# xlite-dev/LeetCUDA

Measured on AMD Instinct MI355X. Metric: achieved fp16 TFLOPS vs MI355X MFMA peak: HGEMM 8192^3; FA-2 fwd S=4096 D=128, higher is better.
Workload: dtype f16 (fp32 MFMA accumulate)

## Files before the change

### include/lc_diag.h

```cpp
#ifndef LC_DIAG_H_
#define LC_DIAG_H_

#ifdef __cplusplus
extern "C" {
#endif

int lc_probe_mfma16(const void* a16x32, const void* b16x32, float* d16x16, void* stream);
int lc_probe_mfma32(const void* a32x16, const void* b32x16, float* d32x32, void* stream);
int lc_probe_tr16(const void* src_64x4_u16, void* dst_64x4_u16, void* stream);
int lc_probe_coissue(int filler, int k, int mode, void* out_u64x16, void* stream);
int lc_probe_attn_mix(int waves, int mix, void* out_u64x16, void* stream);
int lc_diag_attn_w4u_stamps(const void* Q, const void* K, const void* V, void* O, void* lse, int B, int H, int N, int nsplit, void* out_u64x16,
                            void* stream);
int lc_probe_mfma_form(int form, void* out_u64x16, void* stream);
int lc_probe_mfma_war(int delay, int kind, int queued, const void* a32x16, const void* b32x16, float* d32x32,
                      void* stream);

int lc_diag_pollute(unsigned pattern, int what, void* stream);

int lc_diag_attn_w4i(int abl, const void* Q, const void* K, const void* V, void* O, int B, int H, int N, int D, void* stream);

int lc_probe_mid256(const void* A, const void* B, void* C, int M, int N, int K, int b_kn, int panel_w, void* stream);

#ifdef __cplusplus
}
#endif
#endif
```

### leetcuda_amd/build.py

```python
from __future__ import annotations

import argparse
import json
import os
import shutil
import subprocess
import sys
from pathlib import Path

ROOT = Path(__file__).resolve().parent.parent
PKG = ROOT / "leetcuda_amd"
CSRC = PKG / "csrc"
LIBDIR = PKG / "lib"
ORACLE = ROOT / "oracle"
ROCM = Path(os.environ.get("ROCM_PATH", "/opt/rocm"))

LIB_NAME = "libleetcuda_amd.so"
ORACLE_NAME = "liblc_oracle.so"


def _newer(target: Path, sources) -> bool:
    if not target.exists():
        return False
    t = target.stat().st_mtime
    return all(Path(s).stat().st_mtime <= t for s in sources)


def _digest(paths, extra="") -> str:
    import hashlib
    h = hashlib.sha256(extra.encode())
    for q in sorted(Path(x) for x in paths):
        h.update(str(q.relative_to(ROOT) if q.is_relative_to(ROOT) else q).encode())
        h.update(q.read_bytes() if q.exists() else b"<missing>")
    return h.hexdigest()


def _stamps() -> dict:
    try:
        return json.loads((LIBDIR / "stamps.json").read_text())
    except Exception:
        return {}


def _fresh(target: Path, key: str, digest: str) -> bool:
    return target.exists() and _stamps().get(key) == digest


def _mark(key: str, digest: str):
    LIBDIR.mkdir(parents=True, exist_ok=True)
    st = _stamps()
    st[key] = digest
    (LIBDIR / "stamps.json").write_text(json.dumps(st, indent=1))


def _run(cmd, **kw):
    print("[build]", " ".join(str(c) for c in cmd), flush=True)
    subprocess.run([str(c) for c in cmd], check=True, **kw)


def hipcc() -> str:
    exe = shutil.which("hipcc") or str(ROCM / "bin" / "hipcc")
    if not Path(exe).exists():
        raise RuntimeError("hipcc not found: the MI355X kernels cannot be built")
    return exe


def _flags():
    diag = os.environ.get("LC_DIAG") == "1"
    return ["--offload-arch=gfx950", "-O3", "-std=c++17", "-fPIC", "-Wno-unused-result", "-fno-honor-nans",
            "-mno-amdgpu-ieee", *(["-DLC_DIAG"] if diag else []), f"-I{ROOT / 'include'}"]


def _portable(flags):
    return [str(f).replace(str(ROOT), "$ROOT") for f in flags]


def _stamp_ok(stamp: Path, flags) -> bool:
    try:
        return json.loads(stamp.read_text())["flags"] == _portable(flags)
    except Exception:
        return False


def _unit_deps(dep: Path):
    txt = dep.read_text().replace("\\\n", " ")
    return [Path(d) for d in (txt.split(":", 1)[1].split() if ":" in txt else [])]


def _unit_digest(dep: Path, flags) -> str:
    import hashlib
    h = hashlib.sha256(" ".join(_portable(flags)).encode())
    for q in sorted(_unit_deps(dep), key=lambda x: (x.name, str(x))):
        h.update(q.name.encode())
        h.update(q.read_bytes() if q.exists() else b"<missing>")
    return h.hexdigest()


def _unit_current(obj: Path, asm, dep: Path, flags) -> bool:
    if not obj.exists() or not dep.exists() or (asm is not None and not asm.exists()):
        return False
    deps = _unit_deps(dep)
    if not deps or not all(d.exists() for d in deps):
        return False
    have = _stamps().get("unit:" + obj.stem)
    if have is None:
        return False
    return have == _unit_digest(dep, flags)


def build_abi(force: bool = False, audit: bool = True) -> Path:
    LIBDIR.mkdir(parents=True, exist_ok=True)
    out = LIBDIR / LIB_NAME
    stamp = LIBDIR / "build_stamp.json"
    srcs = sorted(CSRC.glob("*.hip")) + sorted(CSRC.glob("*.h")) + sorted(CSRC.glob("*.inc"))
    srcs.append(ROOT / "include" / "lc_abi.h")
    srcs.append(PKG / "isa_audit.py")
    srcs.append(ROOT / "tools" / "gen_hgemm_w4y.py")
    srcs.append(ROOT / "tools" / "gen_attn_w4i.py")
    srcs.append(ROOT / "tools" / "gen_gemm_fp8_w4k.py")
    srcs.append(ROOT / "tools" / "gen_attn_bigd7.py")
    flags = _flags()
    gen = subprocess.run([sys.executable, str(ROOT / "tools" / "gen_hgemm_w4y.py"), "--check"], capture_output=True, text=True)
    if gen.returncode != 0:
        raise RuntimeError("generated sources are stale: " + gen.stderr.strip())
    for script in ("gen_attn_w4i.py", "gen_gemm_fp8_w4k.py", "gen_attn_bigd7.py"):
        gen = subprocess.run([sys.executable, str(ROOT / "tools" / script), "--check"], capture_output=True, text=True)
        if gen.returncode != 0:
            raise RuntimeError("generated sources are stale: " + gen.stderr.strip())
    if os.environ.get("LC_DIAG") == "1":
        subprocess.run([sys.executable, str(ROOT / "tools" / "gen_hgemm_w4y.py"), "--diag", str(LIBDIR / "gen")], check=True)
        flags = flags + [f"-I{LIBDIR / 'gen'}"]
    dg = _digest(srcs, " ".join(_portable(flags)))
    if not force and _fresh(out, "abi", dg) and _stamp_ok(stamp, flags):
        return out
    objdir = LIBDIR / "obj"
    objdir.mkdir(exist_ok=True)
    units = [CSRC / "lc_abi.hip"] + sorted(CSRC.glob("tu_*.hip"))
    for old in list(objdir.glob("tu_*.*")):
        if old.suffix in (".o", ".s", ".d") and not (CSRC / (old.stem + ".hip")).exists():
            old.unlink()
    flags_ok = _stamp_ok(stamp, flags)
    procs = []
    for u in units:
        obj = objdir / (u.stem + ".o")
        asm = objdir / (u.stem + ".s")
        dep = objdir / (u.stem + ".d")
        if not force and flags_ok and _unit_current(obj, asm if audit else None, dep, flags):
            procs.append((u, obj, None))
            continue
        for stale in (obj, asm):
            if stale.exists():
                stale.unlink()
        cmd = [hipcc(), *flags, "-MD", "-MF", str(dep), "-c", "-o", str(obj), str(u)]
        print("[build] " + " ".join(cmd), flush=True)
        procs.append((u, obj, subprocess.Popen(cmd, stdout=subprocess.PIPE, stderr=subprocess.STDOUT, text=True)))
        if audit:
            cmd = [hipcc(), *flags, "-S", "--cuda-device-only", "-Wno-unused-command-line-argument", "-o", str(asm), str(u)]
            procs.append((u, None, subprocess.Popen(cmd, stdout=subprocess.PIPE, stderr=subprocess.STDOUT, text=True)))
    objs = []
    for u, obj, pr in procs:
        if pr is not None:
            log, _ = pr.communicate()
            if pr.returncode != 0:
                sys.stdout.write(log[-8000:])
                raise subprocess.CalledProcessError(pr.returncode, pr.args)
        if obj is not None:
            objs.append(obj)
            if pr is not None:
                _mark("unit:" + obj.stem, _unit_digest(objdir / (obj.stem + ".d"), flags))
    if audit:
        from leetcuda_amd import isa_audit
        reps, bad = isa_audit.audit_files([objdir / (u.stem + ".s") for u in units])
        for r in reps:
            print(f"[audit] {r.name}: vgpr {r.vgpr_count} agpr {r.agpr_count} scratch {r.scratch} "
                  f"asm loads {r.asm_loads} compiler v_accvgpr {r.compiler_accvgpr}", flush=True)
        (objdir / "isa_audit.json").write_text(json.dumps(
            [{"kernel": r.name, "vgpr": r.vgpr_count, "agpr": r.agpr_count, "scratch": r.scratch,
              "asm_loads": r.asm_loads, "compiler_accvgpr": r.compiler_accvgpr, "violations": r.violations}
             for r in reps], indent=1))
        if bad:
            if out.exists():
                out.unlink()
            raise RuntimeError("ISA audit failed (leetcuda_amd/isa_audit.py):\n  " + "\n  ".join(bad))
    _run([hipcc(), "--offload-arch=gfx950", "-shared", "-fPIC", "-o", out, *objs, "-ldl"])
    stamp.write_text(json.dumps({"flags": _portable(flags)}))
    _mark("abi", dg)
    return out


def build_diag(force: bool = False) -> Path:
    LIBDIR.mkdir(parents=True, exist_ok=True)
    out = LIBDIR / "liblc_diag.so"
    srcs = sorted((CSRC / "diag").glob("*.hip")) + [CSRC / "lc_common.h", ROOT / "include" / "lc_diag.h", CSRC / "attn_w4i.hip", CSRC / "attn_w4u.hip", CSRC / "attn_w4u_body.inc", CSRC / "attn_mp.h", CSRC / "attn_fwd.hip", CSRC / "attn_fwd_body.inc",
                                                     CSRC / "hgemm_mid.hip", ROOT / "tools" / "gen_attn_w4i.py"]
    dg = _digest(srcs)
    if not force and _fresh(out, "diag", dg):
        return out
    gen = LIBDIR / "gen"
    subprocess.run([sys.executable, str(ROOT / "tools" / "gen_attn_w4i.py"), "--diag", str(gen)], check=True)
    sys.path.insert(0, str(ROOT / "tools"))
    try:
        import gen_attn_w4i
        abls = gen_attn_w4i.ABLATIONS
    finally:
        sys.path.pop(0)
    objdir = LIBDIR / "obj"
    objdir.mkdir(exist_ok=True)
    base = [hipcc(), "--offload-arch=gfx950", "-O3", "-std=c++17", "-fPIC", "-Wno-unused-result", "-Wno-inline-asm",
            "-fno-honor-nans", "-mno-amdgpu-ieee", f"-I{ROOT / 'include'}", f"-I{gen}", f"-I{CSRC}"]
    jobs = [(objdir / "diag_main.o", [*base, "-c", "-o", objdir / "diag_main.o", CSRC / "diag" / "lc_diag.hip"]),
            (objdir / "diag_w4u_stamps.o", [*base, "-c", "-o", objdir / "diag_w4u_stamps.o", CSRC / "diag" / "attn_w4u_stamps.hip"]),
            (objdir / "diag_mid256.o", [*base, "-c", "-o", objdir / "diag_mid256.o", CSRC / "diag" / "mid256_probe.hip"])]
    for k in abls:
        o = objdir / f"diag_w4i_abl{k}.o"
        jobs.append((o, [*base, f"-DW4I_ABL={k}", f'-DW4I_INC32="attn_w4i_d32_abl{k}.inc"', f'-DW4I_INC64="attn_w4i_d64_abl{k}.inc"', f'-DW4I_INC96="attn_w4i_d96_abl{k}.inc"', f'-DW4I_INC128="attn_w4i_d128_abl{k}.inc"',
                         "-c", "-o", o, CSRC / "diag" / "attn_w4i_abl.hip"]))
    procs = []
    for o, cmd in jobs:
        print("[build]", " ".join(str(c) for c in cmd), flush=True)
        procs.append((o, subprocess.Popen([str(c) for c in cmd], stdout=subprocess.PIPE, stderr=subprocess.STDOUT, text=True)))
    for o, pr in procs:
        log, _ = pr.communicate()
        if pr.returncode != 0:
            sys.stdout.write(log[-6000:])
            raise subprocess.CalledProcessError(pr.returncode, pr.args)
    _run([hipcc(), "--offload-arch=gfx950", "-shared", "-fPIC", "-o", out, *[o for o, _ in jobs]])
    _mark("diag", dg)
    return out


def build_cpp_bench(force: bool = False) -> Path:
    d = ROOT / "tools" / "cpp"
    out = d / "hgemm_bench.bin"
    build_abi(False)
    dg = _digest([d / "hgemm_bench.cpp", d / "Makefile", ROOT / "include" / "lc_abi.h"])
    if not force and _fresh(out, "cpp_bench", dg):
        return out
    _run(["make", "-C", d, "-B"])
    _mark("cpp_bench", dg)
    return out


def build_oracle(force: bool = False) -> Path:
    out = ORACLE / ORACLE_NAME
    srcs = [ORACLE / "lc_oracle.c", ORACLE / "lc_oracle.h"]
    dg = _digest(srcs)
    if not force and _fresh(out, "oracle", dg):
        return out
    cc = shutil.which("gcc") or "cc"
    _run([cc, "-O3", "-mavx2", "-mfma", "-fopenmp", "-fPIC", "-shared", "-std=c11", "-o", out,
          ORACLE / "lc_oracle.c", "-lm"])
    _mark("oracle", dg)
    return out


def build_torch_ext(force: bool = False):
    import sysconfig

    import torch
    from torch.utils import cpp_extension

    suffix = sysconfig.get_config_var("EXT_SUFFIX") or ".so"
    outs = []
    abi = build_abi(force=False)
    inc = [f"-I{p}" for p in cpp_extension.include_paths()] + [f"-I{ROOT / 'include'}"]
    inc += [f"-I{sysconfig.get_paths()['include']}", f"-I{ROCM / 'include'}"]
    torch_lib = Path(torch.__file__).parent / "lib"
    cxx = shutil.which("g++") or "c++"
    for name in ("toy_hgemm", "flash_attn_lib"):
        src = CSRC / "torch" / f"{name}.cpp"
        out = PKG / f"{name}{suffix}"
        dg = _digest([src, CSRC / "torch" / "torch_shim.h", ROOT / "include" / "lc_abi.h"], extra="rpath: $ORIGIN/lib, $ORIGIN/leetcuda_amd/lib")
        if not force and _fresh(out, f"torch_{name}", dg):
            outs.append(out)
            continue
        cmd = [cxx, "-O2", "-std=c++17", "-fPIC", "-shared", "-D__HIP_PLATFORM_AMD__=1",
               "-DUSE_ROCM=1", f"-DTORCH_EXTENSION_NAME={name}", "-DTORCH_API_INCLUDE_EXTENSION_H",
               f"-D_GLIBCXX_USE_CXX11_ABI={int(torch._C._GLIBCXX_USE_CXX11_ABI)}", *inc, src, "-o", out,
               f"-L{LIBDIR}", "-lleetcuda_amd", "-Wl,-rpath,$ORIGIN/lib", "-Wl,-rpath,$ORIGIN/leetcuda_amd/lib", f"-L{torch_lib}",
               "-lc10", "-lc10_hip", "-ltorch", "-ltorch_cpu", "-ltorch_hip", "-ltorch_python",
               f"-Wl,-rpath,{torch_lib}"]
        _run(cmd)
        _mark(f"torch_{name}", dg)
        outs.append(out)
    return outs


def build_all(force: bool = False, torch_ext: bool = True):
    abi = build_abi(force)
    build_diag(force)
    build_cpp_bench(force)
    orc = build_oracle(force)
    ext = build_torch_ext(force) if torch_ext else []
    return abi, orc, ext


if __name__ == "__main__":
    ap = argparse.ArgumentParser()
    ap.add_argument("--force", action="store_true")
    ap.add_argument("--no-torch-ext", action="store_true")
    a = ap.parse_args()
    res = build_all(a.force, not a.no_torch_ext)
    print("[build] ok:", res)
    sys.exit(0)
```

### leetcuda_amd/capi.py

```python
from __future__ import annotations

import ctypes as C
import os
from pathlib import Path

_PKG = Path(__file__).resolve().parent
LIB_PATH = _PKG / "lib" / "libleetcuda_amd.so"
DIAG_LIB_PATH = _PKG / "lib" / "liblc_diag.so"

LC_OK, LC_ERR_ARG, LC_ERR_SHAPE, LC_ERR_HEADDIM, LC_ERR_LAUNCH, LC_ERR_VENDOR, LC_ERR_DEVICE = 0, -1, -2, -3, -4, -5, -6
LAYOUT_NN, LAYOUT_TN = 0, 1
HGEMM_AUTO, HGEMM_MFMA256, HGEMM_GENERIC, HGEMM_MFMA256P2, HGEMM_MFMA128 = 0, 1, 3, 4, 6
HGEMM_VALU_NAIVE, HGEMM_VALU_SLICED_K, HGEMM_VALU_T8X8_X4, HGEMM_VALU_T16X8_K32 = 20, 21, 22, 30
HGEMM_MFMA256W4B, HGEMM_MFMA256W4C, HGEMM_MFMA256W4X, HGEMM_MFMA256W4Y = 9, 10, 12, 13
HGEMM_MID = 14
HGEMM_EDGE = 15
HGEMM_RAGGED = 16
HGEMM_KPAD = 17
ATTN_SPLIT_Q, ATTN_SHARED_QKV, ATTN_SHARED_KV, ATTN_TILING_QK, ATTN_TILING_QKV, ATTN_SPLIT_KV = range(6)
ATTN_CAUSAL, ATTN_V_TRANSPOSED = 1, 2

_vp, _i, _cp, _fp, _ip = C.c_void_p, C.c_int, C.c_char_p, C.POINTER(C.c_float), C.POINTER(C.c_int)
SYMBOLS = {
    "lc_abi_version": (_i, []),
    "lc_status_string": (_cp, [_i]),
    "lc_device_check": (_i, [_ip]),
    "lc_build_info": (_cp, [_ip]),
    "lc_tune_set": (_i, [_cp, _i]),
    "lc_tune_get": (_i, [_cp, _ip, _ip]),
    "lc_tune_count": (_i, []),
    "lc_tune_key": (_cp, [_i]),
    "lc_tune_calibrate": (_i, [_vp, _fp]),
    "lc_workspace_release": (C.c_size_t, []),
    "lc_workspace_bytes": (C.c_size_t, []),
    "lc_hgemm_f16": (_i, [_vp, _vp, _vp, _i, _i, _i, _i, _i, _i, _i, _vp]),
    "lc_vendor_init": (_i, []),
    "lc_vendor_destroy": (_i, []),
    "lc_hgemm_vendor_f16": (_i, [_vp, _vp, _vp, _i, _i, _i, _i, _vp]),
    "lc_gemm_fp8_e4m3": (_i, [_vp, _vp, _vp, _i, _i, _i, C.c_float, _i, _vp]),
    "lc_mxfp8_pack_scales": (_i, [_vp, _vp, _i, _i, _vp]),
    "lc_gemm_mxfp8": (_i, [_vp, _vp, _vp, _vp, _vp, _i, _i, _i, C.c_float, _i, _vp]),
    "lc_hgemm_call": (_i, [_cp, _vp, _vp, _vp, _i, _i, _i, _i, _i, _i, _vp]),
    "lc_hgemm_entry_count": (_i, []),
    "lc_hgemm_entry_name": (_cp, [_i]),
    "lc_hgemm_entry_info": (_i, [_cp, _ip, _ip]),
    "lc_attn_fwd_f16": (_i, [_vp, _vp, _vp, _vp, _i, _i, _i, _i, _i, _i, _i, _i, _vp]),
    "lc_attn_fwd_bf16": (_i, [_vp, _vp, _vp, _vp, _i, _i, _i, _i, _vp]),
    "lc_attn_fwd_f16_ex": (_i, [_vp, _vp, _vp, _vp, _i, _i, _i, _i, _i, _vp]),
    "lc_attn_call": (_i, [_cp, _vp, _vp, _vp, _vp, _i, _i, _i, _i, _i, _vp]),
    "lc_attn_entry_count": (_i, []),
    "lc_attn_entry_name": (_cp, [_i]),
    "lc_attn_entry_info": (_i, [_cp, _ip, _ip, _ip, _ip, _ip, _ip]),
    "lc_hgemm_time": (_i, [_vp, _vp, _vp, _i, _i, _i, _i, _i, _i, _i, _i, _i, _vp, _fp]),
    "lc_attn_time": (_i, [_vp, _vp, _vp, _vp, _i, _i, _i, _i, _i, _i, _i, _i, _i, _vp, _fp]),
    "lc_hgemm_kernel_name": (_i, [_i, _i, _i, _i, _i, _cp, _i]),
    "lc_attn_kernel_name": (_i, [_i, _i, _i, _i, _cp, _i]),
    "lc_attn_kernel_name_bh": (_i, [_i, _i, _i, _i, _i, _cp, _i]),
    "lc_attn_kernel_name_ex": (_i, [_i, _i, _i, _i, _cp, _i]),
    "lc_attn_slowpath_stats": (_i, [C.POINTER(C.c_uint), _i]),
    "lc_timer_start": (_i, [_vp, C.POINTER(_vp)]),
    "lc_timer_stop": (_i, [_vp, _fp]),
    "lc_clock_probe": (_i, [_vp, _vp]),
}
DIAG_SYMBOLS = {
    "lc_probe_mid256": (_i, [_vp, _vp, _vp, _i, _i, _i, _i, _i, _vp]),
    "lc_probe_mfma16": (_i, [_vp, _vp, _vp, _vp]),
    "lc_probe_mfma32": (_i, [_vp, _vp, _vp, _vp]),
    "lc_probe_tr16": (_i, [_vp, _vp, _vp]),
    "lc_probe_coissue": (_i, [_i, _i, _i, _vp, _vp]),
    "lc_probe_attn_mix": (_i, [_i, _i, _vp, _vp]),
    "lc_probe_mfma_form": (_i, [_i, _vp, _vp]),
    "lc_probe_mfma_war": (_i, [_i, _i, _i, _vp, _vp, _vp, _vp]),
    "lc_diag_pollute": (_i, [C.c_uint, _i, _vp]),
    "lc_diag_attn_w4i": (_i, [_i, _vp, _vp, _vp, _vp, _i, _i, _i, _i, _vp]),
    "lc_diag_attn_w4u_stamps": (_i, [_vp, _vp, _vp, _vp, _vp, _i, _i, _i, _i, _vp, _vp]),
}

_lib = None
_diag = None


class LcError(RuntimeError):
    def __init__(self, status: int, what: str):
        self.status = status
        super().__init__(f"{what}: {status_string(status)} (lc_status {status})")


def load() -> C.CDLL:
    global _lib
    if _lib is not None:
        return _lib
    if not LIB_PATH.exists():
        raise RuntimeError(
            f"{LIB_PATH} is missing: build it with `python -m leetcuda_amd.build` "
            "(there is no CPU or PyTorch fallback for the HIP kernels)")
    try:
        import torch
        tl = Path(torch.__file__).parent / "lib" / "libhipblaslt.so"
        if tl.exists() and os.environ.get("LC_VENDOR_SYSTEM_HIPBLASLT", "0") != "1":
            C.CDLL(str(tl), mode=C.RTLD_GLOBAL)
    except Exception:
        pass
    lib = C.CDLL(str(LIB_PATH), mode=C.RTLD_GLOBAL)
    for name, (res, args) in SYMBOLS.items():
        fn = getattr(lib, name)
        fn.restype, fn.argtypes = res, args
    _lib = lib
    return lib


def load_diag() -> C.CDLL:
    global _diag
    if _diag is not None:
        return _diag
    if not DIAG_LIB_PATH.exists():
        raise RuntimeError(f"{DIAG_LIB_PATH} is missing: build it with `python -m leetcuda_amd.build`")
    import torch
    lib = C.CDLL(str(DIAG_LIB_PATH), mode=C.RTLD_GLOBAL)
    for name, (res, args) in DIAG_SYMBOLS.items():
        fn = getattr(lib, name)
        fn.restype, fn.argtypes = res, args
    _diag = lib
    return lib


def build_info():
    d = C.c_int(0)
    return load().lc_build_info(C.byref(d)).decode(), bool(d.value)


def require_production():
    info, diag = build_info()
    if diag:
        raise RuntimeError(f"libleetcuda_amd.so is a DIAGNOSIS build ({info}); rebuild with "
                           "`python -m leetcuda_amd.build --force` (LC_DIAG unset)")


def status_string(status: int) -> str:
    return load().lc_status_string(status).decode()


def check(status: int, what: str):
    if status != LC_OK:
        raise LcError(status, what)


def _ptr(t) -> int:
    return t.data_ptr()


def _stream() -> int:
    import torch
    return torch.cuda.current_stream().cuda_stream


def _shape_err(what: str):
    raise RuntimeError(f"Tensor size mismatch! ({what})")


def _gemm_dims(a, b, c, layout=LAYOUT_NN, b_is_nk=False):
    if a.dim() != 2 or b.dim() != 2 or c.dim() != 2:
        _shape_err("2-D tensors expected")
    M, K = a.shape
    N = c.shape[1]
    if c.shape[0] != M:
        _shape_err(f"c {tuple(c.shape)} vs a {tuple(a.shape)}")
    if b_is_nk:
        ok = tuple(b.shape) == (N, K)
    elif layout == LAYOUT_TN:
        ok = tuple(b.shape) in ((K, N), (N, K))
    else:
        ok = tuple(b.shape) == (K, N)
    if not ok:
        _shape_err(f"b {tuple(b.shape)} vs K={K}, N={N}")
    return M, N, K


def _attn_dims(q, k, v, o, v_transposed=False):
    if q.dim() != 4:
        _shape_err("4-D [B,H,N,D] tensors expected")
    B, H, N, D = q.shape
    vshape = (B, H, D, N) if v_transposed else (B, H, N, D)
    if tuple(k.shape) != (B, H, N, D) or tuple(o.shape) != (B, H, N, D) or tuple(v.shape) != vshape:
        _shape_err(f"q {tuple(q.shape)} k {tuple(k.shape)} v {tuple(v.shape)} o {tuple(o.shape)}")
    return B, H, N, D


def _need_gpu(*tensors):
    for t in tensors:
        if not t.is_cuda:
            raise RuntimeError("leetcuda_amd: tensor must live on the MI355X (no CPU path)")
        if not t.is_contiguous():
            raise RuntimeError("leetcuda_amd: tensor must be contiguous")


def tune(key: str, value: int):
    check(load().lc_tune_set(key.encode(), value), f"lc_tune_set({key})")


def tune_get(key: str):
    v, d = C.c_int(0), C.c_int(0)
    check(load().lc_tune_get(key.encode(), C.byref(v), C.byref(d)), f"lc_tune_get({key})")
    return v.value, d.value


def tune_items():
    lib = load()
    out = {}
    for i in range(lib.lc_tune_count()):
        k = lib.lc_tune_key(i)
        if k:
            out[k.decode()] = tune_get(k.decode())
    return out


def tune_calibrate():
    out = (C.c_float * 4)()
    rc = load().lc_tune_calibrate(_stream(), out)
    if rc not in (LC_OK, LC_ERR_ARG):
        check(rc, "lc_tune_calibrate")
    return {"adopted": rc == LC_OK, "tau128_us": out[0], "tau64_us": out[1], "x0_us": out[2], "bytes_per_us": out[3]}


def workspace_bytes() -> int:
    return int(load().lc_workspace_bytes())


def workspace_release() -> int:
    return int(load().lc_workspace_release())


def device_check() -> int:
    n = C.c_int(0)
    check(load().lc_device_check(C.byref(n)), "lc_device_check")
    return n.value


def hgemm(a, b, c, layout=LAYOUT_NN, variant=HGEMM_AUTO, stages=2, swizzle_stride=1):
    import torch
    _need_gpu(a, b, c)
    assert a.dtype == b.dtype == c.dtype == torch.half
    M, N, K = _gemm_dims(a, b, c, layout)
    check(load().lc_hgemm_f16(_ptr(a), _ptr(b), _ptr(c), M, N, K, layout, variant, stages, swizzle_stride,
                              _stream()), "lc_hgemm_f16")
    return c


def gemm_fp8(a8, b8_nk, c, alpha=1.0, swizzle_stride=1):
    _need_gpu(a8, b8_nk, c)
    M, N, K = _gemm_dims(a8, b8_nk, c, b_is_nk=True)
    check(load().lc_gemm_fp8_e4m3(_ptr(a8), _ptr(b8_nk), _ptr(c), M, N, K, float(alpha), swizzle_stride, _stream()),
          "lc_gemm_fp8_e4m3")
    return c


def mxfp8_pack_scales(s):
    import torch
    _need_gpu(s)
    assert s.dtype == torch.uint8 and s.dim() == 2 and s.is_contiguous()
    rows, kb = s.shape
    p = torch.empty(rows * kb, dtype=torch.uint8, device=s.device)
    check(load().lc_mxfp8_pack_scales(_ptr(s), _ptr(p), rows, kb * 32, _stream()), "lc_mxfp8_pack_scales")
    return p


def gemm_mxfp8(a8, pa, b8_nk, pb, c, alpha=1.0, swizzle_stride=1):
    _need_gpu(a8, b8_nk, c, pa, pb)
    M, N, K = _gemm_dims(a8, b8_nk, c, b_is_nk=True)
    assert pa.numel() == M * K // 32 and pb.numel() == N * K // 32
    check(load().lc_gemm_mxfp8(_ptr(a8), _ptr(pa), _ptr(b8_nk), _ptr(pb), _ptr(c), M, N, K, float(alpha), swizzle_stride, _stream()),
          "lc_gemm_mxfp8")
    return c


def hgemm_call(entry: str, a, b, c, stages=2, swizzle=False, swizzle_stride=1):
    _need_gpu(a, b, c)
    lay = C.c_int(LAYOUT_NN)
    load().lc_hgemm_entry_info(entry.encode(), C.byref(lay), None)
    M, N, K = _gemm_dims(a, b, c, lay.value)
    check(load().lc_hgemm_call(entry.encode(), _ptr(a), _ptr(b), _ptr(c), M, N, K, stages, int(swizzle),
                               swizzle_stride, _stream()), entry)
    return c


def hgemm_vendor(a, b, c, layout=LAYOUT_NN):
    _need_gpu(a, b, c)
    M, N, K = _gemm_dims(a, b, c, layout)
    check(load().lc_hgemm_vendor_f16(_ptr(a), _ptr(b), _ptr(c), M, N, K, layout, _stream()),
          "lc_hgemm_vendor_f16")
    return c


def vendor_init():
    check(load().lc_vendor_init(), "lc_vendor_init")


def vendor_destroy():
    check(load().lc_vendor_destroy(), "lc_vendor_destroy")


def hgemm_time(a, b, c, layout=LAYOUT_NN, variant=HGEMM_AUTO, stages=2, swizzle_stride=1, warmup=2,
               iters=10) -> float:
    _need_gpu(a, b, c)
    M, N, K = _gemm_dims(a, b, c, layout)
    ms = C.c_float(0)
    check(load().lc_hgemm_time(_ptr(a), _ptr(b), _ptr(c), M, N, K, layout, variant, stages, swizzle_stride,
                               warmup, iters, _stream(), C.byref(ms)), "lc_hgemm_time")
    return ms.value


def hgemm_entries():
    lib = load()
    out = []
    for i in range(lib.lc_hgemm_entry_count()):
        name = lib.lc_hgemm_entry_name(i)
        lay, na = C.c_int(), C.c_int()
        lib.lc_hgemm_entry_info(name, C.byref(lay), C.byref(na))
        out.append((name.decode(), lay.value, na.value))
    return out


def attn_fwd(q, k, v, o, v_transposed=False, family=ATTN_SPLIT_Q, acc_f32=False, stages=2, causal=False):
    import torch
    _need_gpu(q, k, v, o)
    assert q.dtype == k.dtype == v.dtype == o.dtype == torch.half
    B, H, N, D = _attn_dims(q, k, v, o, v_transposed)
    if causal:
        flags = ATTN_CAUSAL | (ATTN_V_TRANSPOSED if v_transposed else 0)
        check(load().lc_attn_fwd_f16_ex(_ptr(q), _ptr(k), _ptr(v), _ptr(o), B, H, N, D, flags, _stream()), "lc_attn_fwd_f16_ex")
        return o
    check(load().lc_attn_fwd_f16(_ptr(q), _ptr(k), _ptr(v), _ptr(o), B, H, N, D, int(v_transposed), family,
                                 int(acc_f32), stages, _stream()), "lc_attn_fwd_f16")
    return o


def attn_fwd_bf16(q, k, v, o):
    import torch
    _need_gpu(q, k, v, o)
    assert q.dtype == k.dtype == v.dtype == o.dtype == torch.bfloat16
    B, H, N, D = _attn_dims(q, k, v, o)
    check(load().lc_attn_fwd_bf16(_ptr(q), _ptr(k), _ptr(v), _ptr(o), B, H, N, D, _stream()), "lc_attn_fwd_bf16")
    return o


def attn_call(entry: str, q, k, v, o, stages=2):
    _need_gpu(q, k, v, o)
    vt = C.c_int(0)
    load().lc_attn_entry_info(entry.encode(), None, C.byref(vt), None, None, None, None)
    B, H, N, D = _attn_dims(q, k, v, o, bool(vt.value))
    check(load().lc_attn_call(entry.encode(), _ptr(q), _ptr(k), _ptr(v), _ptr(o), B, H, N, D, stages,
                              _stream()), entry)
    return o


def attn_time(q, k, v, o, v_transposed=False, family=ATTN_SPLIT_Q, stages=2, warmup=1, iters=5) -> float:
    _need_gpu(q, k, v, o)
    B, H, N, D = _attn_dims(q, k, v, o, v_transposed)
    ms = C.c_float(0)
    check(load().lc_attn_time(_ptr(q), _ptr(k), _ptr(v), _ptr(o), B, H, N, D, int(v_transposed), family,
                              stages, warmup, iters, _stream(), C.byref(ms)), "lc_attn_time")
    return ms.value


def attn_entries():
    lib = load()
    out = []
    for i in range(lib.lc_attn_entry_count()):
        name = lib.lc_attn_entry_name(i)
        v = [C.c_int() for _ in range(6)]
        lib.lc_attn_entry_info(name, *[C.byref(x) for x in v])
        out.append((name.decode(),) + tuple(x.value for x in v))
    return out


class Timer:

    def __enter__(self):
        self._t = C.c_void_p()
        check(load().lc_timer_start(_stream(), C.byref(self._t)), "lc_timer_start")
        self.ms = None
        return self

    def __exit__(self, et, ev, tb):
        ms = C.c_float(0)
        rc = load().lc_timer_stop(self._t, C.byref(ms))
        if et is None:
            check(rc, "lc_timer_stop")
            self.ms = ms.value
        return False


def hgemm_kernel_name(M, N, K, layout=LAYOUT_NN, variant=HGEMM_AUTO) -> str:
    buf = C.create_string_buffer(128)
    check(load().lc_hgemm_kernel_name(M, N, K, layout, variant, buf, 128), "lc_hgemm_kernel_name")
    return buf.value.decode()


def attn_slowpath_stats(reset=True):
    import struct
    out = (C.c_uint * 4)()
    check(load().lc_attn_slowpath_stats(out, int(reset)), "lc_attn_slowpath_stats")
    return [out[0], out[1], out[2], struct.unpack("f", struct.pack("I", out[3]))[0]]


def attn_kernel_name(N, D, v_transposed=False, bf16=False, bh=None, causal=False) -> str:
    buf = C.create_string_buffer(128)
    if causal:
        assert not bf16, "causal attention is fp16 only"
        flags = ATTN_CAUSAL | (ATTN_V_TRANSPOSED if v_transposed else 0)
        check(load().lc_attn_kernel_name_ex(int(bh) if bh else -1, N, D, flags, buf, 128), "lc_attn_kernel_name_ex")
        return buf.value.decode()
    check(load().lc_attn_kernel_name_bh(int(bh) if bh else -1, N, D, int(v_transposed), int(bf16), buf, 128), "lc_attn_kernel_name_bh")
    return buf.value.decode()


def clock_probe(out_u64x2):
    check(load().lc_clock_probe(_ptr(out_u64x2), _stream()), "lc_clock_probe")
```

### leetcuda_amd/csrc/hgemm_w4y.hip

```cpp
#pragma once
#include "hgemm_w4x.hip"

namespace lc {

struct W4yNNSrc {
  const char* ub;
  unsigned b_off[2];
  unsigned bq, bkt;
};
LC_DEVINL void w4y_nn_src_init(W4yNNSrc& s, const half_t* B, int n0, int N, int wave, int lane) {
  const int pp = lane & 15, kr = lane >> 4;
#pragma unroll
  for (int par = 0; par < 2; ++par) {
    const int pair = (pp >> 1) ^ ((kr << 1) | par);
    s.b_off[par] = (unsigned)kr * (unsigned)N * 2u + (unsigned)((pair * 2 + (pp & 1)) * 16);
  }
  s.ub = (const char*)(B + (size_t)(wave * 16) * N + n0);
  s.bq = (unsigned)N * 8u;
  s.bkt = (unsigned)N * 128u;
}

template <bool ALPHA = false>
LC_DEVINL void w4y_epilogue_b2(char* slot, half_t* C, int N, int m0, int n0, int wave, int wr, int wc, int lane, float alpha = 1.f) {
  asm volatile("" : "+v"(lane));
  const int r16 = lane & 15, kg = lane >> 4;
  char* stg = slot + wave * (32 * 256);
  half_t* cw = C + (size_t)(m0 + wr * 128) * N + n0 + wc * 128;
  static_for<4>([&](auto qc) {
    constexpr int q = decltype(qc)::value;
    static_for<4>([&](auto gc) {
      constexpr int ih = decltype(gc)::value >> 1, j0 = 4 * (decltype(gc)::value & 1);
      constexpr int blk = 8 * (2 * q + ih) + j0;
      float x[16];
      acc_read16<4 * blk, 4 * (blk + 1), 4 * (blk + 2), 4 * (blk + 3)>(x);
#pragma unroll
      for (int jj = 0; jj < 4; ++jj) {
        const int j = j0 + jj;
        half4_t h;
        if constexpr (ALPHA) {
          h[0] = (half_t)(alpha * x[4 * jj + 0]);
          h[1] = (half_t)(alpha * x[4 * jj + 1]);
          h[2] = (half_t)(alpha * x[4 * jj + 2]);
          h[3] = (half_t)(alpha * x[4 * jj + 3]);
        } else {
          h[0] = (half_t)x[4 * jj + 0];
          h[1] = (half_t)x[4 * jj + 1];
          h[2] = (half_t)x[4 * jj + 2];
          h[3] = (half_t)x[4 * jj + 3];
        }
        *(half4_t*)(stg + (16 * ih + r16) * 256 + (((2 * j + (kg >> 1)) ^ r16) * 16) + 8 * (kg & 1)) = h;
      }
    });
    asm volatile("s_waitcnt lgkmcnt(0)" ::: "memory");
#pragma unroll
    for (int it = 0; it < 8; ++it) {
      const int row = it * 4 + (lane >> 4);
      const u32x4_t v = *(const u32x4_t*)(stg + row * 256 + (((lane & 15) ^ (row & 15)) * 16));
      *(u32x4_t*)(cw + (size_t)(q * 32 + row) * N + (lane & 15) * 8) = v;
    }
    asm volatile("s_waitcnt lgkmcnt(0)" ::: "memory");
  });
}

template <int BLK0, int BLK1>
LC_DEVINL void w4y_tail_mfma2(half8_t b0, half8_t b1, half8_t a) {
  asm volatile("s_nop 1\n\tv_mfma_f32_16x16x32_f16 a[%3:%4], %0, %2, a[%3:%4]\n\tv_mfma_f32_16x16x32_f16 a[%5:%6], %1, %2, a[%5:%6]"
               :: "v"(b0), "v"(b1), "v"(a), "n"(BLK0 * 4), "n"(BLK0 * 4 + 3), "n"(BLK1 * 4), "n"(BLK1 * 4 + 3)
               : LC_AGPR_ALL);
}
template <bool B_KN>
LC_DEVINL void w4y_k_tail(const half_t* __restrict__ A, const half_t* __restrict__ B, int N, int K, int k0, int mw, int nw, int lane) {
  asm volatile("" : "+v"(lane), "+s"(N), "+s"(K));
  const int r16 = lane & 15, kg = lane >> 4;
  const half_t* ap = A + ((size_t)(mw + r16) * K + k0 + 8 * kg);
  half8_t xb[8];
  if constexpr (!B_KN) {
    const half_t* bp = B + ((size_t)(nw + r16) * K + k0 + 8 * kg);
#pragma unroll
    for (int j = 0; j < 8; ++j) xb[j] = *(const half8_t*)(bp + (size_t)16 * j * K);
  } else {
    const half_t* bp = B + ((size_t)(k0 + 8 * kg) * N + nw + r16);
#pragma unroll
    for (int e = 0; e < 8; ++e) {
      const half_t* be = bp + (size_t)e * N;
#pragma unroll
      for (int j = 0; j < 8; ++j) xb[j][e] = be[16 * j];
    }
  }
  static_for<8>([&](auto ic) {
    constexpr int i = decltype(ic)::value;
    const half8_t xa = *(const half8_t*)(ap + (size_t)16 * i * K);
    static_for<4>([&](auto jc) {
      constexpr int jp = decltype(jc)::value;
      w4y_tail_mfma2<8 * i + 2 * jp, 8 * i + 2 * jp + 1>(xb[2 * jp], xb[2 * jp + 1], xa);
    });
  });
}

template <bool B_KN, int SCHED>
__global__ __launch_bounds__(256) void hgemm_w4y_kernel(const half_t* __restrict__ A, const half_t* __restrict__ B,
                                                       half_t* __restrict__ C, int M, int N, int K, int tiles_m,
                                                       int tiles_n, int panel_w, int stagger, int ntiles) {
  extern __shared__ __attribute__((aligned(16))) char smem[];
  const int lane = threadIdx.x & 63;
  const int wave = wave_id();
  const int wr = wave >> 1, wc = wave & 1;

  int vb = __builtin_amdgcn_readfirstlane((int)blockIdx.x);
  const int vstride = __builtin_amdgcn_readfirstlane((int)gridDim.x);
  const int nvb = ntiles > 0 ? ntiles : vstride;
  const int KT = K / BK;

  W4Src<false> src;
  w4_src_init<false>(src, A, B, 0, 0, N, K, wave, lane);
  src.a_off[0] = src.a_off[1] = (wave & 1) ? src.a_off[1] : src.a_off[0];
  src.a_blk = (size_t)32 * K * 2;
  W4yNNSrc nsrc;
  if constexpr (B_KN) w4y_nn_src_init(nsrc, B, 0, N, wave, lane);

  struct TileCtx {
    int m0, n0;
    const char* ua;
    const char* ub;
    uint32_t stg;
  };
  auto tile_ctx = [&](int v) -> TileCtx {
    const TileCoord tc = block_tile(v, nvb, tiles_m, tiles_n, panel_w);
    TileCtx c;
    c.m0 = tc.tm * BM;
    c.n0 = tc.tn * BN;
    c.ua = (const char*)(A + (size_t)(c.m0 + wave * 8) * K);
    c.ub = B_KN ? (const char*)(B + (size_t)(wave * 16) * N + c.n0) : (const char*)(B + (size_t)(c.n0 + wave * 8) * K);
    const int cx = stagger & 15, cm = (stagger >> 4) & 15, cn = (stagger >> 8) & 15, step = (stagger >> 12) & 0xff, mask = (stagger >> 20) & 0x7f;
    const int idx = cx * (v & 7) + cm * __builtin_amdgcn_readfirstlane(tc.tm) + cn * __builtin_amdgcn_readfirstlane(tc.tn);
    c.stg = (uint32_t)__builtin_amdgcn_readfirstlane((int)((unsigned)((idx & mask) * step) % (unsigned)KT));
    return c;
  };
  auto a_slot = [&](int t) -> char* { return smem + (t & 1) * TILE_BYTES; };
  auto b_slot = [&](int bi) -> char* { return smem + (2 + bi) * TILE_BYTES; };
  auto issue_prologue = [&](const TileCtx& c) {
    const buf_rsrc_t ra = make_rsrc(c.ua), rb = make_rsrc(c.ub);
    auto piece = [&](int g, int t, char* slot) {
      int te = (t < KT ? t : KT - 1) + (int)c.stg;
      if (te >= KT) te -= KT;
      if (g < 8) {
        blds16(ra, src.a_off[0], (unsigned)((size_t)g * src.a_blk + (size_t)te * src.a_kt), slot + g * 4096 + wave * 1024);
      } else if constexpr (!B_KN) {
        blds16(rb, src.a_off[0], (unsigned)((size_t)(g - 8) * src.a_blk + (size_t)te * src.b_kt),
               slot + (g - 8) * 4096 + wave * 1024);
      } else {
        const int p = g - 8, h = p >> 2, p2 = p & 3;
        blds16(rb, nsrc.b_off[(p2 >> 1) & 1], (unsigned)p2 * nsrc.bq + 256u * h + (unsigned)te * nsrc.bkt,
               slot + h * HALF_BYTES + (wave * 4 + p2) * 1024);
      }
    };
#pragma unroll
    for (int g = 8; g < 16; ++g) piece(g, 0, b_slot(0));
#pragma unroll
    for (int g = 0; g < 8; ++g) piece(g, 0, a_slot(0));
#pragma unroll
    for (int g = 8; g < 16; ++g) piece(g, 1, b_slot(1));
#pragma unroll
    for (int g = 0; g < 8; ++g) piece(g, 1, a_slot(1));
  };

  W4xFrag fr;
  w4x_frag_init(fr, wr, wc, lane);

  TileCtx cur = tile_ctx(vb);
  issue_prologue(cur);
  for (;;) {
  static_for<256>([&](auto r) { w4_acc_zero<decltype(r)::value>(); });
  LC_VMCNT(16);
  pp_barrier();
  const int m0 = cur.m0, n0 = cur.n0;
  const uint32_t w4y_stg = cur.stg;
  const char* ubp = cur.ub;

  {
    const uint64_t pa = (uint64_t)cur.ua, pb = (uint64_t)ubp;
    const u32x4_t w4y_ra = {(uint32_t)__builtin_amdgcn_readfirstlane((uint32_t)pa),
                            (uint32_t)__builtin_amdgcn_readfirstlane((uint32_t)(pa >> 32)) & 0xffffu, 0x7fffffffu, 0x00020000u};
    const u32x4_t w4y_rb = {(uint32_t)__builtin_amdgcn_readfirstlane((uint32_t)pb),
                            (uint32_t)__builtin_amdgcn_readfirstlane((uint32_t)(pb >> 32)) & 0xffffu, 0x7fffffffu, 0x00020000u};
    const uint32_t w4y_a0 = __builtin_amdgcn_readfirstlane(lds_addr32(smem));
    const uint32_t w4y_wv = (uint32_t)wave * 1024u;
    const uint32_t w4y_blk = __builtin_amdgcn_readfirstlane((uint32_t)src.a_blk);
    const uint32_t w4y_ao0 = src.a_off[0], w4y_ao1 = src.a_off[1];
    uint32_t w4y_t, w4y_acur, w4y_anxt, w4y_b0, w4y_b1, w4y_b2, w4y_soff, w4y_t2off, w4y_tmp, w4y_swp;
    if constexpr (B_KN) {
      const uint32_t w4y_wvb = (uint32_t)wave * 4096u;
      const uint32_t w4y_bq = __builtin_amdgcn_readfirstlane(nsrc.bq), w4y_bkt = __builtin_amdgcn_readfirstlane(nsrc.bkt);
      const uint32_t w4y_bo0 = nsrc.b_off[0], w4y_bo1 = nsrc.b_off[1];
      const int ti = lane & 15, tg = lane >> 4;
      const uint32_t w4y_bk = (uint32_t)(wc * HALF_BYTES + (8 * tg + (ti >> 2)) * 256 + (ti & 3) * 8);
      const uint32_t w4y_key = (uint32_t)(((ti >> 2) << 1) | (tg & 1));
      uint32_t w4y_t2offb;
#include "hgemm_w4y_loop_nn.inc"
    } else if constexpr (SCHED == 0) {
#include "hgemm_w4y_loop0.inc"
    } else if constexpr (SCHED == 1) {
#include "hgemm_w4y_loop1.inc"
#ifdef LC_DIAG
    } else if constexpr (SCHED == 3) {
#include "hgemm_w4y_loop3.inc"
    } else if constexpr (SCHED == 4) {
#include "hgemm_w4y_loop4.inc"
    } else if constexpr (SCHED == 5) {
#include "hgemm_w4y_loop5.inc"
#endif
    } else {
#include "hgemm_w4y_loop2.inc"
    }
  }
  if (K & 32) w4y_k_tail<B_KN>(A, B, N, K, KT * BK, m0 + wr * 128, n0 + wc * 128, lane);
  w4_mfma_drain();
  __syncthreads();
  const int vbn = __builtin_amdgcn_readfirstlane(vb + vstride);
  const bool has_next = ntiles > 0 && vbn < ntiles;
  TileCtx nxt = cur;
  if (has_next) {
    nxt = tile_ctx(vbn);
    issue_prologue(nxt);
  }
  w4y_epilogue_b2(smem + 4 * TILE_BYTES, C, N, m0, n0, wave, wr, wc, lane);
  if (!has_next) break;
  vb = vbn;
  cur = nxt;
  }
}

}
```

### leetcuda_amd/csrc/lc_knobs.inc

```
#ifndef LC_KNOB_SNAP
#define LC_KNOB_SNAP LC_KNOB
#endif
LC_KNOB_SNAP(attn_nw, 0, ok_attn_nw, false)
LC_KNOB_SNAP(attn_walk, 0, ok_03, false)
LC_KNOB_SNAP(attn_split, 0, ok_split, false)
LC_KNOB_SNAP(attn_causal_order, 0, ok_02, false)
LC_KNOB(attn_bigd_map, 0, ok_02, false)
LC_KNOB(attn_bigd_stagger, 0, ok_02, false)
LC_KNOB_SNAP(attn_d1024, 0, ok_span8, false)
LC_KNOB_SNAP(attn_w4i_sched, 1, ok_01, false)
LC_KNOB(fp8_mx, 3, ok_03, false)
LC_KNOB_SNAP(attn_d512, 0, ok_04, false)
LC_KNOB_SNAP(w4y_sched, 2, ok_w4y_sched, false)
LC_KNOB(hgemm_persist, 1, ok_01, false)
LC_KNOB(hgemm_stagger, 0, ok_stagger, false)
LC_KNOB_SNAP(hgemm_tail, 1, ok_04, false)
LC_KNOB_SNAP(hgemm_tail_tile, 0, ok_02, false)
LC_KNOB_SNAP(hgemm_ragged, 0, ok_01, false)
LC_KNOB_SNAP(hgemm_ragged_fork, 0, ok_02, false)
LC_KNOB_SNAP(hgemm_ragged_tile, 0, ok_ragged_tile, false)
LC_KNOB_SNAP(hgemm_kpad, 0, ok_02, false)
LC_KNOB_SNAP(hgemm_mid_splitk, 0, ok_08, false)
LC_KNOB_SNAP(hgemm_128w, 0, ok_02, false)
LC_KNOB_SNAP(rule_cus, 0, ok_rule_cus, false)
LC_KNOB_SNAP(attn_calib, 0, ok_01, false)
LC_KNOB_SNAP(hgemm_mid, 0, ok_mid, false)
LC_KNOB_SNAP(hgemm_mid_ns, 0, ok_mid_ns, false)
LC_KNOB_SNAP(hgemm_splitk, 0, ok_08, false)
LC_KNOB_SNAP(hgemm_raster, 0, ok_02, false)
LC_KNOB_SNAP(hgemm_auto, LC_HGEMM_MFMA256W4Y, ok_auto, false)
LC_KNOB_SNAP(w4_abl, 0, ok_any, true)
LC_KNOB_SNAP(hgemm_stamps, 0, ok_01, true)
LC_KNOB_SNAP(attn_ablate, 0, ok_any, true)
#undef LC_KNOB
#undef LC_KNOB_SNAP
```

### leetcuda_amd/csrc/lc_launch.h

```cpp
#pragma once
#include <hip/hip_runtime.h>

#include <atomic>
#include <mutex>
#include <utility>
#include <vector>

#include "../../include/lc_abi.h"
#include "lc_common.h"

namespace lc {

inline int launch_guard() { return hipPeekAtLastError() == hipSuccess ? LC_OK : LC_ERR_LAUNCH; }
inline int check_launch() { return hipGetLastError() == hipSuccess ? LC_OK : LC_ERR_LAUNCH; }

template <typename KernelT>
int set_dyn_lds(KernelT kernel, int bytes) {
  static std::mutex mu;
  static std::vector<std::pair<const void*, int>> done;
  const void* fn = reinterpret_cast<const void*>(kernel);
  int dev = 0;
  if (hipGetDevice(&dev) != hipSuccess) return LC_ERR_DEVICE;
  std::lock_guard<std::mutex> g(mu);
  for (const auto& d : done)
    if (d.first == fn && d.second == dev) return LC_OK;
  if (hipFuncSetAttribute(fn, hipFuncAttributeMaxDynamicSharedMemorySize, bytes) != hipSuccess)
    return LC_ERR_LAUNCH;
  done.emplace_back(fn, dev);
  return LC_OK;
}

inline int device_cu_count() {
  static std::mutex mu;
  static int cache[64] = {};
  int dev = 0;
  if (hipGetDevice(&dev) != hipSuccess || dev < 0 || dev >= 64) return 256;
  std::lock_guard<std::mutex> g(mu);
  if (cache[dev] == 0) {
    int v = 0;
    if (hipDeviceGetAttribute(&v, hipDeviceAttributeMultiprocessorCount, dev) != hipSuccess || v <= 0) v = 256;
    cache[dev] = v;
  }
  return cache[dev];
}

struct WorkspaceLease {
  std::unique_lock<std::mutex> lock;
  void* ptr = nullptr;
};
constexpr size_t kWorkspaceCapBytes = (size_t)1 << 30;
struct WorkspaceEntry { hipStream_t st; void* p; size_t bytes; unsigned long long tick; };
struct WorkspacePool {
  std::mutex mu;
  std::vector<WorkspaceEntry> entries;
  unsigned long long tick = 0;
};
inline WorkspacePool& workspace_pool(int dev) {
  static WorkspacePool pools[64];
  return pools[(dev >= 0 && dev < 64) ? dev : 0];
}
struct RelaxedCaptureMode {
  hipStreamCaptureMode prev = hipStreamCaptureModeRelaxed;
  bool ok;
  RelaxedCaptureMode() { ok = hipThreadExchangeStreamCaptureMode(&prev) == hipSuccess; if (!ok) (void)hipGetLastError(); }
  ~RelaxedCaptureMode() { if (ok) (void)hipThreadExchangeStreamCaptureMode(&prev); }
};
inline bool& workspace_held_by_this_thread() {
  static thread_local bool held = false;
  return held;
}
inline WorkspaceLease stream_workspace(hipStream_t st, size_t bytes) {
  WorkspaceLease lease;
  if (workspace_held_by_this_thread()) return lease;
  int dev = 0;
  if (hipGetDevice(&dev) != hipSuccess) {
    (void)hipGetLastError();
    return lease;
  }
  WorkspacePool& pool = workspace_pool(dev);
  lease.lock = std::unique_lock<std::mutex>(pool.mu);
  if (bytes == 0 || bytes > kWorkspaceCapBytes) return lease;
  bytes = (bytes + ((size_t)1 << 22) - 1) & ~(((size_t)1 << 22) - 1);
  WorkspaceEntry* e = nullptr;
  for (auto& x : pool.entries)
    if (x.st == st) e = &x;
  if (e && e->bytes >= bytes) {
    e->tick = ++pool.tick;
    lease.ptr = e->p;
    return lease;
  }
  RelaxedCaptureMode relaxed;
  if (!e && pool.entries.size() >= 16) {
    size_t lru = 0;
    for (size_t i = 1; i < pool.entries.size(); ++i)
      if (pool.entries[i].tick < pool.entries[lru].tick) lru = i;
    (void)hipFree(pool.entries[lru].p);
    pool.entries.erase(pool.entries.begin() + lru);
  }
  if (e) {
    size_t grown = e->bytes + e->bytes / 2;
    grown = (grown + ((size_t)1 << 22) - 1) & ~(((size_t)1 << 22) - 1);
    if (grown > bytes && grown <= kWorkspaceCapBytes) bytes = grown;
    (void)hipFree(e->p);
    e->p = nullptr;
    e->bytes = 0;
  }
  void* p = nullptr;
  if (hipMalloc(&p, bytes) != hipSuccess || !p) {
    (void)hipGetLastError();
    if (e) pool.entries.erase(pool.entries.begin() + (e - pool.entries.data()));
    return lease;
  }
  if (e) {
    e->p = p;
    e->bytes = bytes;
    e->tick = ++pool.tick;
  } else {
    pool.entries.push_back(WorkspaceEntry{st, p, bytes, ++pool.tick});
  }
  lease.ptr = p;
  return lease;
}
inline size_t workspace_release_all() {
  size_t freed = 0;
  int cur = 0;
  const bool have_cur = hipGetDevice(&cur) == hipSuccess;
  RelaxedCaptureMode relaxed;
  for (int dev = 0; dev < 64; ++dev) {
    WorkspacePool& pool = workspace_pool(dev);
    std::lock_guard<std::mutex> g(pool.mu);
    if (pool.entries.empty()) continue;
    if (hipSetDevice(dev) != hipSuccess) {
      (void)hipGetLastError();
      continue;
    }
    for (auto& x : pool.entries) {
      (void)hipFree(x.p);
      freed += x.bytes;
    }
    pool.entries.clear();
  }
  if (have_cur) (void)hipSetDevice(cur);
  return freed;
}
inline size_t workspace_cached_bytes() {
  size_t n = 0;
  for (int dev = 0; dev < 64; ++dev) {
    WorkspacePool& pool = workspace_pool(dev);
    std::lock_guard<std::mutex> g(pool.mu);
    for (auto& x : pool.entries) n += x.bytes;
  }
  return n;
}
inline bool stream_is_capturing(hipStream_t st) {
  hipStreamCaptureStatus cap = hipStreamCaptureStatusNone;
  if (hipStreamIsCapturing(st, &cap) != hipSuccess) {
    (void)hipGetLastError();
    return true;
  }
  return cap != hipStreamCaptureStatusNone;
}

using tune_t = std::atomic<int>;
extern tune_t g_tune_attn_bigd_stagger;
extern tune_t g_tune_attn_bigd_map;
extern tune_t g_tune_hgemm_persist;
extern tune_t g_tune_hgemm_stagger;
constexpr int STAGGER_OFF = 1 << 27;
inline int stagger_arg(int kt) {
  const int knob = g_tune_hgemm_stagger;
  if (knob == STAGGER_OFF) return 0;
  if (knob != 0) return knob;
  const int step = kt / 8;
  return 1 | (step < 1 ? 1 : step > 255 ? 255 : step) << 12 | 7 << 20;
}

struct HgemmPlan;
struct AttnPlan;
int launch_hgemm(const HgemmPlan& p, const half_t* A, const half_t* B, half_t* C, int M, int N, int K, bool b_kn, int swizzle_stride, hipStream_t st);
int launch_attn_plan(const AttnPlan& p, const half_t* Q, const half_t* K, const half_t* V, half_t* O, int B, int H, int N, int D, bool vt, bool bf16,
                     hipStream_t st);
int launch_clock_probe(unsigned long long* out_u64x2, hipStream_t st);
int launch_hgemm_mid(const half_t* A, const half_t* B, half_t* C, int M, int N, int K, bool b_kn, int tmw, int tnw, int ns, int pw,
                     hipStream_t st, float* part = nullptr, int ks = 1);
int launch_hgemm_mid_edge(const half_t* A, const half_t* B, half_t* C, int M, int N, int K, bool b_kn, int tmw, int tnw, int ns, int Mi, int Ni, hipStream_t st);
size_t launch_hgemm_mid_edge_sk_floats(int M, int N, int tmw, int ks);
int launch_hgemm_mid_edge_sk(const half_t* A, const half_t* B, half_t* C, int M, int N, int K, bool b_kn, int tmw, int ks, float* part, hipStream_t st);
int launch_hgemm_mid_rem(const half_t* A, const half_t* B, half_t* C, int M, int N, int K, bool b_kn, int tmw, int ns, int tiles_m256,
                         int tiles_n256, int pw256, int rem_base, int rem_tiles, hipStream_t st);
int launch_w4_family(const half_t* A, const half_t* B, half_t* C, int M, int N, int K, int variant, int sched, int stamps, int abl, bool b_kn,
                     int tiles_m, int tiles_n, int panel_w, int nblk, hipStream_t st);
int launch_valu_rung(const half_t* A, const half_t* B, half_t* C, int M, int N, int K, int rung, hipStream_t st);
void valu_rung_tile(int rung, int* tm, int* tn, int* tk);
const char* valu_rung_kernel_name(int rung);
int launch_attn_w4u_d128(const half_t* Q, const half_t* K, const half_t* V, half_t* O, int B, int H, int N, int walk, int nsplit, hipStream_t st);
int launch_attn_w4u_d128t(const half_t* Q, const half_t* K, const half_t* V, half_t* O, int B, int H, int N, int walk, int nsplit, hipStream_t st);
int launch_attn_w4u_d64(const half_t* Q, const half_t* K, const half_t* V, half_t* O, int B, int H, int N, int walk, int nsplit, hipStream_t st);
int launch_attn_w4u_d64t(const half_t* Q, const half_t* K, const half_t* V, half_t* O, int B, int H, int N, int walk, int nsplit, hipStream_t st);
int launch_attn_w4u_causal_d128(const half_t* Q, const half_t* K, const half_t* V, half_t* O, int B, int H, int N, int order, hipStream_t st);
int launch_attn_w4u_causal_d128t(const half_t* Q, const half_t* K, const half_t* V, half_t* O, int B, int H, int N, int order, hipStream_t st);
int launch_attn_w4u_causal_d64(const half_t* Q, const half_t* K, const half_t* V, half_t* O, int B, int H, int N, int order, hipStream_t st);
int launch_attn_w4u_causal_d64t(const half_t* Q, const half_t* K, const half_t* V, half_t* O, int B, int H, int N, int order, hipStream_t st);
int diag_attn_slowpath_u_d128(unsigned* out4, int reset);
int diag_attn_slowpath_u_d128t(unsigned* out4, int reset);
int diag_attn_slowpath_u_d64(unsigned* out4, int reset);
int diag_attn_slowpath_u_d64t(unsigned* out4, int reset);
int launch_attn_w4i(const half_t* Q, const half_t* K, const half_t* V, half_t* O, int B, int H, int N, int D, int sched, hipStream_t st);
int diag_attn_slowpath_g(unsigned* out4, int reset);
int launch_attn_bigd2(const half_t* Q, const half_t* K, const half_t* V, half_t* O, int B, int H, int N, int D, bool bf16, bool bigd3,
                      hipStream_t st);
int launch_attn_bigd4(const half_t* Q, const half_t* K, const half_t* V, half_t* O, int B, int H, int N, int span8, hipStream_t st);
int launch_attn_bigd2_vt(const half_t* Q, const half_t* K, const half_t* V, half_t* O, int B, int H, int N, int D, hipStream_t st);
int launch_attn_bigd6(const half_t* Q, const half_t* K, const half_t* V, half_t* O, int B, int H, int N, bool bf16, hipStream_t st);
int launch_attn_bigd7(const half_t* Q, const half_t* K, const half_t* V, half_t* O, int B, int H, int N, bool bf16, hipStream_t st);
int launch_attn_bigd7_vt(const half_t* Q, const half_t* K, const half_t* V, half_t* O, int B, int H, int N, hipStream_t st);
int launch_gemm_fp8(const uint8_t* A, const uint8_t* B, half_t* C, int M, int N, int K, float alpha, int tiles_m,
                    int tiles_n, int panel_w, int mx, hipStream_t st);
bool gemm_fp8_w4k_fits(int K);
int launch_gemm_fp8_w4k(const uint8_t* A, const uint8_t* B, half_t* C, int M, int N, int K, float alpha, int tiles_m, int tiles_n,
                        int panel_w, hipStream_t st);
int launch_gemm_mxfp8(const uint8_t* A, const uint32_t* PA, const uint8_t* B, const uint32_t* PB, half_t* C, int M, int N, int K,
                      float alpha, int tiles_m, int tiles_n, int panel_w, hipStream_t st);
int launch_mx_pack_scales(const uint8_t* S, uint32_t* P, int rows, int K, hipStream_t st);

}
```

### leetcuda_amd/csrc/tu_w4.hip

```cpp
#include "lc_launch.h"
#include "hgemm_w4y.hip"

namespace lc {
namespace {
template <bool B_KN, bool BUF, int DG>
int launch_w4_one(const half_t* A, const half_t* B, half_t* C, int M, int N, int K, int tiles_m, int tiles_n, int pw,
                  hipStream_t st) {
  auto kern = hgemm_w4b_kernel<B_KN, BUF, DG>;
  if (int rc = set_dyn_lds(kern, W4B_LDS)) return rc;
  hipLaunchKernelGGL(kern, dim3(tiles_m * tiles_n), dim3(256), W4B_LDS, st, A, B, C, M, N, K, tiles_m, tiles_n, pw);
  return check_launch();
}

template <bool B_KN, int Y>
int launch_w4x_one(const half_t* A, const half_t* B, half_t* C, int M, int N, int K, int tiles_m, int tiles_n, int pw,
                   int nblk_arg, hipStream_t st) {
  auto kern = [] {
    if constexpr (Y < 0) return hgemm_w4x_kernel<B_KN>;
    else return hgemm_w4y_kernel<B_KN, Y>;
  }();
  if (int rc = set_dyn_lds(kern, W4B_LDS)) return rc;
  const int nblk = nblk_arg > 0 ? nblk_arg : tiles_m * tiles_n;
  if constexpr (Y < 0) {
    hipLaunchKernelGGL(kern, dim3(nblk), dim3(256), W4B_LDS, st, A, B, C, M, N, K, tiles_m, tiles_n, pw);
  } else {
    const int ncu = device_cu_count();
    const bool persist = g_tune_hgemm_persist != 0 && nblk > ncu && nblk % ncu == 0;
    hipLaunchKernelGGL(kern, dim3(persist ? ncu : nblk), dim3(256), W4B_LDS, st, A, B, C, M, N, K, tiles_m, tiles_n, pw,
                       stagger_arg(K / BK), persist ? nblk : 0);
  }
  return check_launch();
}

template <bool B_KN>
int launch_w4_t(const half_t* A, const half_t* B, half_t* C, int M, int N, int K, int variant, int sched, int stamps, int abl, int tiles_m,
                int tiles_n, int pw, int nblk, hipStream_t st) {
#ifdef LC_DIAG
  if (variant == LC_HGEMM_MFMA256W4C && stamps)
    return launch_w4_one<B_KN, true, 1>(A, B, C, M, N, K, tiles_m, tiles_n, pw, st);
  if (variant == LC_HGEMM_MFMA256W4C && abl) {
    switch (abl) {
      case 2: return launch_w4_one<B_KN, true, 2>(A, B, C, M, N, K, tiles_m, tiles_n, pw, st);
      case 4: return launch_w4_one<B_KN, true, 4>(A, B, C, M, N, K, tiles_m, tiles_n, pw, st);
      case 6: return launch_w4_one<B_KN, true, 6>(A, B, C, M, N, K, tiles_m, tiles_n, pw, st);
      case 8: return launch_w4_one<B_KN, true, 8>(A, B, C, M, N, K, tiles_m, tiles_n, pw, st);
      case 14: return launch_w4_one<B_KN, true, 14>(A, B, C, M, N, K, tiles_m, tiles_n, pw, st);
      default: return LC_ERR_ARG;
    }
  }
#endif
  if constexpr (!B_KN) {
    if (variant == LC_HGEMM_MFMA256W4X) return launch_w4x_one<B_KN, -1>(A, B, C, M, N, K, tiles_m, tiles_n, pw, nblk, st);
    if (variant == LC_HGEMM_MFMA256W4Y) {
      if (sched == 0) return launch_w4x_one<B_KN, 0>(A, B, C, M, N, K, tiles_m, tiles_n, pw, nblk, st);
      if (sched == 1) return launch_w4x_one<B_KN, 1>(A, B, C, M, N, K, tiles_m, tiles_n, pw, nblk, st);
#ifdef LC_DIAG
      if (sched == 3) return launch_w4x_one<B_KN, 3>(A, B, C, M, N, K, tiles_m, tiles_n, pw, nblk, st);
      if (sched == 4) return launch_w4x_one<B_KN, 4>(A, B, C, M, N, K, tiles_m, tiles_n, pw, nblk, st);
      if (sched == 5) return launch_w4x_one<B_KN, 5>(A, B, C, M, N, K, tiles_m, tiles_n, pw, nblk, st);
#endif
      return launch_w4x_one<B_KN, 2>(A, B, C, M, N, K, tiles_m, tiles_n, pw, nblk, st);
    }
  } else {
    if (variant == LC_HGEMM_MFMA256W4Y) return launch_w4x_one<B_KN, 1>(A, B, C, M, N, K, tiles_m, tiles_n, pw, nblk, st);
  }
  if (variant == LC_HGEMM_MFMA256W4C || variant == LC_HGEMM_MFMA256W4X || variant == LC_HGEMM_MFMA256W4Y)
    return launch_w4_one<B_KN, true, 0>(A, B, C, M, N, K, tiles_m, tiles_n, pw, st);
  return launch_w4_one<B_KN, false, 0>(A, B, C, M, N, K, tiles_m, tiles_n, pw, st);
}
}

int launch_w4_family(const half_t* A, const half_t* B, half_t* C, int M, int N, int K, int variant, int sched, int stamps, int abl, bool b_kn,
                     int tiles_m, int tiles_n, int panel_w, int nblk, hipStream_t st) {
  return b_kn ? launch_w4_t<true>(A, B, C, M, N, K, variant, sched, stamps, abl, tiles_m, tiles_n, panel_w, nblk, st)
              : launch_w4_t<false>(A, B, C, M, N, K, variant, sched, stamps, abl, tiles_m, tiles_n, panel_w, nblk, st);
}
}
```

Measured before the change: 1518.

## Carry next tile's global-to-LDS prefetch across tiles in persistent W4Y HGEMM

Adds a CARRY variant of the persistent TN W4Y HGEMM kernel. Its hand-written asm main loop issues the next tile's buffer_load-to-LDS prologue from inside the current tile's K loop, so loads are never drained at tile boundaries and the per-tile barrier and prologue bubble disappears. The variant is enabled by default through a new hgemm_carry knob when the launch is persistent and offsets fit in 32 bits. It also adds s_memtime stamp instrumentation and a diagnostic entry point. The cost is added complexity and a register- and LDS-buffer rotation scheme that could introduce hazards.

```diff
diff --git a/include/lc_diag.h b/include/lc_diag.h
--- a/include/lc_diag.h
+++ b/include/lc_diag.h
@@ -12,6 +12,8 @@
 int lc_probe_attn_mix(int waves, int mix, void* out_u64x16, void* stream);
 int lc_diag_attn_w4u_stamps(const void* Q, const void* K, const void* V, void* O, void* lse, int B, int H, int N, int nsplit, void* out_u64x16,
                             void* stream);
+int lc_diag_hgemm_w4y_stamps(const void* A, const void* B, void* C, int M, int N, int K, int panel_w, int stagger, int carry, void* out_u64x128,
+                             void* stream);
 int lc_probe_mfma_form(int form, void* out_u64x16, void* stream);
 int lc_probe_mfma_war(int delay, int kind, int queued, const void* a32x16, const void* b32x16, float* d32x32,
                       void* stream);
diff --git a/leetcuda_amd/build.py b/leetcuda_amd/build.py
--- a/leetcuda_amd/build.py
+++ b/leetcuda_amd/build.py
@@ -192,7 +192,8 @@
     LIBDIR.mkdir(parents=True, exist_ok=True)
     out = LIBDIR / "liblc_diag.so"
     srcs = sorted((CSRC / "diag").glob("*.hip")) + [CSRC / "lc_common.h", ROOT / "include" / "lc_diag.h", CSRC / "attn_w4i.hip", CSRC / "attn_w4u.hip", CSRC / "attn_w4u_body.inc", CSRC / "attn_mp.h", CSRC / "attn_fwd.hip", CSRC / "attn_fwd_body.inc",
-                                                     CSRC / "hgemm_mid.hip", ROOT / "tools" / "gen_attn_w4i.py"]
+                                                     CSRC / "hgemm_mid.hip", ROOT / "tools" / "gen_attn_w4i.py",
+                                                     CSRC / "hgemm_w4y.hip", CSRC / "hgemm_w4x.hip", CSRC / "hgemm_w4.hip", *sorted(CSRC.glob("hgemm_w4y_loop*.inc"))]
     dg = _digest(srcs)
     if not force and _fresh(out, "diag", dg):
         return out
@@ -210,6 +211,7 @@
             "-fno-honor-nans", "-mno-amdgpu-ieee", f"-I{ROOT / 'include'}", f"-I{gen}", f"-I{CSRC}"]
     jobs = [(objdir / "diag_main.o", [*base, "-c", "-o", objdir / "diag_main.o", CSRC / "diag" / "lc_diag.hip"]),
             (objdir / "diag_w4u_stamps.o", [*base, "-c", "-o", objdir / "diag_w4u_stamps.o", CSRC / "diag" / "attn_w4u_stamps.hip"]),
+            (objdir / "diag_w4y_stamps.o", [*base, "-c", "-o", objdir / "diag_w4y_stamps.o", CSRC / "diag" / "hgemm_w4y_stamps.hip"]),
             (objdir / "diag_mid256.o", [*base, "-c", "-o", objdir / "diag_mid256.o", CSRC / "diag" / "mid256_probe.hip"])]
     for k in abls:
         o = objdir / f"diag_w4i_abl{k}.o"
diff --git a/leetcuda_amd/capi.py b/leetcuda_amd/capi.py
--- a/leetcuda_amd/capi.py
+++ b/leetcuda_amd/capi.py
@@ -74,6 +74,7 @@
     "lc_diag_pollute": (_i, [C.c_uint, _i, _vp]),
     "lc_diag_attn_w4i": (_i, [_i, _vp, _vp, _vp, _vp, _i, _i, _i, _i, _vp]),
     "lc_diag_attn_w4u_stamps": (_i, [_vp, _vp, _vp, _vp, _vp, _i, _i, _i, _i, _vp, _vp]),
+    "lc_diag_hgemm_w4y_stamps": (_i, [_vp, _vp, _vp, _i, _i, _i, _i, _i, _i, _vp, _vp]),
 }
 
 _lib = None
diff --git a/leetcuda_amd/csrc/diag/hgemm_w4y_stamps.hip b/leetcuda_amd/csrc/diag/hgemm_w4y_stamps.hip
--- /dev/null
+++ b/leetcuda_amd/csrc/diag/hgemm_w4y_stamps.hip
@@ -0,0 +1,23 @@
+#define W4Y_STAMPS 1
+#define hgemm_w4y_kernel hgemm_w4y_stamped_kernel
+#include "../lc_launch.h"
+#include "../hgemm_w4y.hip"
+
+extern "C" int lc_diag_hgemm_w4y_stamps(const void* A, const void* B, void* C, int M, int N, int K, int panel_w, int stagger, int carry,
+                                        void* out_u64x128, void* stream) {
+  using namespace lc;
+  if (!A || !B || !C || !out_u64x128 || M <= 0 || N <= 0 || M % BM || N % BN || K < 2 * BK || K % BK) return LC_ERR_ARG;
+  if ((size_t)M * K * 2 >= ((size_t)1 << 31) || (size_t)N * K * 2 >= ((size_t)1 << 31)) return LC_ERR_ARG;
+  hipStream_t st = static_cast<hipStream_t>(stream);
+  const int tiles_m = M / BM, tiles_n = N / BN, nblk = tiles_m * tiles_n, ncu = device_cu_count();
+  if (nblk % ncu != 0 || nblk / ncu < 3 || panel_w < 1) return LC_ERR_ARG;
+  auto go = [&](auto kern) -> int {
+    if (int rc = set_dyn_lds(kern, W4B_LDS)) return rc;
+    hipLaunchKernelGGL(kern, dim3(ncu), dim3(256), W4B_LDS, st, (const half_t*)A, (const half_t*)B, (half_t*)C, M, N, K, tiles_m, tiles_n, panel_w,
+                       stagger, nblk);
+    return check_launch();
+  };
+  if (int rc = carry ? go(hgemm_w4y_kernel<false, 2, true>) : go(hgemm_w4y_kernel<false, 2, false>)) return rc;
+  if (hipStreamSynchronize(st) != hipSuccess) return LC_ERR_LAUNCH;
+  return hipMemcpyFromSymbol(out_u64x128, HIP_SYMBOL(g_w4y_stamps), W4Y_STAMP_WGS * 16 * sizeof(unsigned long long)) == hipSuccess ? LC_OK : LC_ERR_LAUNCH;
+}
diff --git a/leetcuda_amd/csrc/hgemm_w4y.hip b/leetcuda_amd/csrc/hgemm_w4y.hip
--- a/leetcuda_amd/csrc/hgemm_w4y.hip
+++ b/leetcuda_amd/csrc/hgemm_w4y.hip
@@ -2,6 +2,25 @@
 #include "hgemm_w4x.hip"
 
 namespace lc {
+
+#ifdef W4Y_STAMPS
+constexpr int W4Y_STAMP_WGS = 8;
+static __device__ unsigned long long g_w4y_stamps[W4Y_STAMP_WGS * 16];
+#define W4Y_STAMP(on, k)                                                                         \
+  do {                                                                                           \
+    if (on) {                                                                                    \
+      unsigned long long t_;                                                                     \
+      __builtin_amdgcn_sched_barrier(0);                                                         \
+      asm volatile("s_memtime %0\n\ts_waitcnt lgkmcnt(0)" : "=s"(t_) :: "memory");               \
+      __builtin_amdgcn_sched_barrier(0);                                                         \
+      if ((threadIdx.x & 63) == 0) g_w4y_stamps[blockIdx.x * 16 + (k)] = t_;                     \
+      if (((k) == 1 || (k) == 11) && (threadIdx.x & 63) == 0)  \
+        g_w4y_stamps[blockIdx.x * 16 + 12 + ((k) == 11)] = __builtin_amdgcn_s_memrealtime();     \
+    }                                                                                            \
+  } while (0)
+#else
+#define W4Y_STAMP(on, k) do { } while (0)
+#endif
 
 struct W4yNNSrc {
   const char* ub;
@@ -21,7 +40,8 @@
 }
 
 template <bool ALPHA = false>
-LC_DEVINL void w4y_epilogue_b2(char* slot, half_t* C, int N, int m0, int n0, int wave, int wr, int wc, int lane, float alpha = 1.f) {
+LC_DEVINL void w4y_epilogue_b2(char* slot, half_t* C, int N, int m0, int n0, int wave, int wr, int wc, int lane, float alpha = 1.f,
+                               bool stamp = false) {
   asm volatile("" : "+v"(lane));
   const int r16 = lane & 15, kg = lane >> 4;
   char* stg = slot + wave * (32 * 256);
@@ -59,6 +79,7 @@
       *(u32x4_t*)(cw + (size_t)(q * 32 + row) * N + (lane & 15) * 8) = v;
     }
     asm volatile("s_waitcnt lgkmcnt(0)" ::: "memory");
+    W4Y_STAMP(stamp, 5 + q);
   });
 }
 
@@ -97,7 +118,7 @@
   });
 }
 
-template <bool B_KN, int SCHED>
+template <bool B_KN, int SCHED, bool CARRY = false>
 __global__ __launch_bounds__(256) void hgemm_w4y_kernel(const half_t* __restrict__ A, const half_t* __restrict__ B,
                                                        half_t* __restrict__ C, int M, int N, int K, int tiles_m,
                                                        int tiles_n, int panel_w, int stagger, int ntiles) {
@@ -166,13 +187,84 @@
 
   W4xFrag fr;
   w4x_frag_init(fr, wr, wc, lane);
+#ifdef W4Y_STAMPS
+  int w4y_ord = 0;
+  const bool w4y_st = wave == 0 && blockIdx.x < W4Y_STAMP_WGS;
+  if (w4y_st && lane == 0) g_w4y_stamps[blockIdx.x * 16 + 14] = __builtin_amdgcn_s_memrealtime();
+#define W4Y_ST(ord, k) W4Y_STAMP(w4y_st && w4y_ord == (ord), k)
+#else
+#define W4Y_ST(ord, k) do { } while (0)
+#endif
+
+  if constexpr (CARRY) {
+    static_assert(!B_KN && SCHED == 2, "the carried stream exists for TN, schedule 2");
+    struct CarryCtx {
+      int m0, n0;
+      uint32_t oa, ob, stg;
+    };
+    auto carry_ctx = [&](const TileCtx& c) -> CarryCtx {
+      return CarryCtx{c.m0, c.n0, (uint32_t)__builtin_amdgcn_readfirstlane((int)((uint32_t)(c.m0 + wave * 8) * (uint32_t)K * 2u)),
+                      (uint32_t)__builtin_amdgcn_readfirstlane((int)((uint32_t)(c.n0 + wave * 8) * (uint32_t)K * 2u)), c.stg};
+    };
+    const uint64_t pa = (uint64_t)A, pb = (uint64_t)B;
+    const u32x4_t w4y_ra = {(uint32_t)__builtin_amdgcn_readfirstlane((uint32_t)pa),
+                            (uint32_t)__builtin_amdgcn_readfirstlane((uint32_t)(pa >> 32)) & 0xffffu, 0x7fffffffu, 0x00020000u};
+    const u32x4_t w4y_rb = {(uint32_t)__builtin_amdgcn_readfirstlane((uint32_t)pb),
+                            (uint32_t)__builtin_amdgcn_readfirstlane((uint32_t)(pb >> 32)) & 0xffffu, 0x7fffffffu, 0x00020000u};
+    const uint32_t w4y_a0 = __builtin_amdgcn_readfirstlane(lds_addr32(smem));
+    const uint32_t w4y_wv = (uint32_t)wave * 1024u;
+    const uint32_t w4y_blk = __builtin_amdgcn_readfirstlane((uint32_t)src.a_blk);
+    const uint32_t w4y_ao0 = src.a_off[0], w4y_ao1 = src.a_off[1];
+    uint32_t w4y_acur = w4y_a0, w4y_anxt = w4y_a0 + TILE_BYTES, w4y_b0 = w4y_a0 + 2 * TILE_BYTES, w4y_b1 = w4y_a0 + 3 * TILE_BYTES,
+             w4y_b2 = w4y_a0 + 4 * TILE_BYTES;
+    const TileCtx first = tile_ctx(vb);
+    issue_prologue(first);
+    CarryCtx cur = carry_ctx(first);
+    LC_VMCNT(16);
+    for (;;) {
+      const int vbn = __builtin_amdgcn_readfirstlane(vb + vstride);
+      const bool has_next = vbn < ntiles;
+      const CarryCtx nxt = has_next ? carry_ctx(tile_ctx(vbn)) : cur;
+      W4Y_ST(2, 9);
+      pp_barrier();
+      W4Y_ST(1, 0);
+      W4Y_ST(2, 10);
+      {
+        const uint32_t w4y_stg = cur.stg, w4y_stgn = nxt.stg, w4y_oa = cur.oa, w4y_ob = cur.ob, w4y_oan = nxt.oa, w4y_obn = nxt.ob;
+        uint32_t w4y_t, w4y_soff, w4y_t2off, w4y_t2offb, w4y_tmp, w4y_swp, w4y_sel, w4y_sela;
+#include "hgemm_w4y_loop2c.inc"
+      }
+      W4Y_ST(1, 1);
+      W4Y_ST(2, 11);
+      if (!has_next) LC_VMCNT(0);
+      if (K & 32) w4y_k_tail<false>(A, B, N, K, KT * BK, cur.m0 + wr * 128, cur.n0 + wc * 128, lane);
+      w4_mfma_drain();
+      W4Y_ST(1, 2);
+#ifdef W4Y_STAMPS
+      w4y_epilogue_b2(smem + (w4y_b2 - w4y_a0), C, N, cur.m0, cur.n0, wave, wr, wc, lane, 1.f, w4y_st && w4y_ord == 1);
+      ++w4y_ord;
+#else
+      w4y_epilogue_b2(smem + (w4y_b2 - w4y_a0), C, N, cur.m0, cur.n0, wave, wr, wc, lane);
+#endif
+      if (!has_next) break;
+      vb = vbn;
+      cur = nxt;
+    }
+#ifdef W4Y_STAMPS
+    if (w4y_st && lane == 0) g_w4y_stamps[blockIdx.x * 16 + 15] = __builtin_amdgcn_s_memrealtime();
+#endif
+    return;
+  }
 
   TileCtx cur = tile_ctx(vb);
   issue_prologue(cur);
   for (;;) {
   static_for<256>([&](auto r) { w4_acc_zero<decltype(r)::value>(); });
+  W4Y_ST(2, 9);
   LC_VMCNT(16);
   pp_barrier();
+  W4Y_ST(1, 0);
+  W4Y_ST(2, 10);
   const int m0 = cur.m0, n0 = cur.n0;
   const uint32_t w4y_stg = cur.stg;
   const char* ubp = cur.ub;
@@ -213,21 +305,34 @@
 #include "hgemm_w4y_loop2.inc"
     }
   }
+  W4Y_ST(1, 1);
+  W4Y_ST(2, 11);
   if (K & 32) w4y_k_tail<B_KN>(A, B, N, K, KT * BK, m0 + wr * 128, n0 + wc * 128, lane);
   w4_mfma_drain();
   __syncthreads();
+  W4Y_ST(1, 2);
   const int vbn = __builtin_amdgcn_readfirstlane(vb + vstride);
   const bool has_next = ntiles > 0 && vbn < ntiles;
   TileCtx nxt = cur;
   if (has_next) {
     nxt = tile_ctx(vbn);
+    W4Y_ST(1, 3);
     issue_prologue(nxt);
-  }
+    W4Y_ST(1, 4);
+  }
+#ifdef W4Y_STAMPS
+  w4y_epilogue_b2(smem + 4 * TILE_BYTES, C, N, m0, n0, wave, wr, wc, lane, 1.f, w4y_st && w4y_ord == 1);
+  ++w4y_ord;
+#else
   w4y_epilogue_b2(smem + 4 * TILE_BYTES, C, N, m0, n0, wave, wr, wc, lane);
+#endif
   if (!has_next) break;
   vb = vbn;
   cur = nxt;
   }
-}
-
-}
+#ifdef W4Y_STAMPS
+  if (w4y_st && lane == 0) g_w4y_stamps[blockIdx.x * 16 + 15] = __builtin_amdgcn_s_memrealtime();
+#endif
+}
+
+}
diff --git a/leetcuda_amd/csrc/hgemm_w4y_loop2c.inc b/leetcuda_amd/csrc/hgemm_w4y_loop2c.inc
--- /dev/null
+++ b/leetcuda_amd/csrc/hgemm_w4y_loop2c.inc
@@ -0,0 +1,527 @@
+asm volatile(
+    "s_mov_b32 %[t], 0\n\t"
+    "v_add_u32_e32 v124, %[acur], %[ar0]\n\t"
+    "v_add_u32_e32 v125, %[b0], %[br0]\n\t"
+    "ds_read_b128 v[128:131], v124 offset:0\n\t"
+    "ds_read_b128 v[132:135], v124 offset:2048\n\t"
+    "ds_read_b128 v[136:139], v124 offset:4096\n\t"
+    "ds_read_b128 v[140:143], v124 offset:6144\n\t"
+    "ds_read_b128 v[144:147], v124 offset:8192\n\t"
+    "ds_read_b128 v[148:151], v124 offset:10240\n\t"
+    "ds_read_b128 v[152:155], v124 offset:12288\n\t"
+    "ds_read_b128 v[156:159], v124 offset:14336\n\t"
+    "ds_read_b128 v[160:163], v125 offset:0\n\t"
+    "ds_read_b128 v[164:167], v125 offset:2048\n\t"
+    "ds_read_b128 v[168:171], v125 offset:4096\n\t"
+    "ds_read_b128 v[172:175], v125 offset:6144\n\t"
+    "ds_read_b128 v[176:179], v125 offset:8192\n\t"
+    "ds_read_b128 v[180:183], v125 offset:10240\n\t"
+    "ds_read_b128 v[184:187], v125 offset:12288\n\t"
+    "ds_read_b128 v[188:191], v125 offset:14336\n\t"
+    "s_mov_b32 %[swp], 2\n\t"
+    "s_cmp_ge_u32 %[swp], %[kt]\n\t"
+    "s_cselect_b32 %[t2off], %[kt], 0\n\t"
+    "s_cselect_b32 %[sel], %[stgn], %[stg]\n\t"
+    "s_cselect_b32 %[t2offb], %[obn], %[ob]\n\t"
+    "s_cselect_b32 %[sela], %[oan], %[oa]\n\t"
+    "s_sub_u32 %[swp], %[swp], %[t2off]\n\t"
+    "s_add_u32 %[swp], %[swp], %[sel]\n\t"
+    "s_cmp_ge_u32 %[swp], %[kt]\n\t"
+    "s_cselect_b32 %[t2off], %[kt], 0\n\t"
+    "s_sub_u32 %[swp], %[swp], %[t2off]\n\t"
+    "s_lshl_b32 %[swp], %[swp], 7\n\t"
+    "s_add_u32 %[t2off], %[swp], %[sela]\n\t"
+    "s_add_u32 %[t2offb], %[swp], %[t2offb]\n\t"
+    "v_add_u32_e32 v124, %[acur], %[ar1]\n\t"
+    "v_add_u32_e32 v125, %[b0], %[br1]\n\t"
+    "s_waitcnt lgkmcnt(0)\n\t"
+    "v_mfma_f32_16x16x32_f16 a[0:3], v[160:163], v[128:131], 0\n\t"
+    "ds_read_b128 v[192:195], v124 offset:0\n\t"
+    "v_mfma_f32_16x16x32_f16 a[4:7], v[164:167], v[128:131], 0\n\t"
+    "v_mfma_f32_16x16x32_f16 a[8:11], v[168:171], v[128:131], 0\n\t"
+    "ds_read_b128 v[196:199], v124 offset:2048\n\t"
+    "s_add_u32 %[tmp], %[b2], %[wv]\n\t"
+    "v_mfma_f32_16x16x32_f16 a[12:15], v[172:175], v[128:131], 0\n\t"
+    "s_add_u32 m0, %[tmp], 0\n\t"
+    "s_mov_b32 %[soff], %[t2offb]\n\t"
+    "v_mfma_f32_16x16x32_f16 a[16:19], v[176:179], v[128:131], 0\n\t"
+    "ds_read_b128 v[200:203], v124 offset:4096\n\t"
+    "buffer_load_dwordx4 %[ao0], %[rb], %[soff] offen lds\n\t"
+    "v_mfma_f32_16x16x32_f16 a[20:23], v[180:183], v[128:131], 0\n\t"
+    "v_mfma_f32_16x16x32_f16 a[24:27], v[184:187], v[128:131], 0\n\t"
+    "ds_read_b128 v[204:207], v124 offset:6144\n\t"
+    "v_mfma_f32_16x16x32_f16 a[28:31], v[188:191], v[128:131], 0\n\t"
+    "v_mfma_f32_16x16x32_f16 a[32:35], v[160:163], v[132:135], 0\n\t"
+    "ds_read_b128 v[208:211], v124 offset:8192\n\t"
+    "v_mfma_f32_16x16x32_f16 a[36:39], v[164:167], v[132:135], 0\n\t"
+    "v_mfma_f32_16x16x32_f16 a[40:43], v[168:171], v[132:135], 0\n\t"
+    "ds_read_b128 v[212:215], v124 offset:10240\n\t"
+    "v_mfma_f32_16x16x32_f16 a[44:47], v[172:175], v[132:135], 0\n\t"
+    "s_add_u32 m0, %[tmp], 4096\n\t"
+    "s_add_u32 %[soff], %[soff], %[blk]\n\t"
+    "v_mfma_f32_16x16x32_f16 a[48:51], v[176:179], v[132:135], 0\n\t"
+    "ds_read_b128 v[216:219], v124 offset:12288\n\t"
+    "buffer_load_dwordx4 %[ao1], %[rb], %[soff] offen lds\n\t"
+    "v_mfma_f32_16x16x32_f16 a[52:55], v[180:183], v[132:135], 0\n\t"
+    "v_mfma_f32_16x16x32_f16 a[56:59], v[184:187], v[132:135], 0\n\t"
+    "ds_read_b128 v[220:223], v124 offset:14336\n\t"
+    "v_mfma_f32_16x16x32_f16 a[60:63], v[188:191], v[132:135], 0\n\t"
+    "v_mfma_f32_16x16x32_f16 a[64:67], v[160:163], v[136:139], 0\n\t"
+    "ds_read_b128 v[224:227], v125 offset:0\n\t"
+    "v_mfma_f32_16x16x32_f16 a[68:71], v[164:167], v[136:139], 0\n\t"
+    "v_mfma_f32_16x16x32_f16 a[72:75], v[168:171], v[136:139], 0\n\t"
+    "ds_read_b128 v[228:231], v125 offset:2048\n\t"
+    "v_mfma_f32_16x16x32_f16 a[76:79], v[172:175], v[136:139], 0\n\t"
+    "s_add_u32 m0, %[tmp], 8192\n\t"
+    "s_add_u32 %[soff], %[soff], %[blk]\n\t"
+    "v_mfma_f32_16x16x32_f16 a[80:83], v[176:179], v[136:139], 0\n\t"
+    "ds_read_b128 v[232:235], v125 offset:4096\n\t"
+    "buffer_load_dwordx4 %[ao0], %[rb], %[soff] offen lds\n\t"
+    "v_mfma_f32_16x16x32_f16 a[84:87], v[180:183], v[136:139], 0\n\t"
+    "v_mfma_f32_16x16x32_f16 a[88:91], v[184:187], v[136:139], 0\n\t"
+    "ds_read_b128 v[236:239], v125 offset:6144\n\t"
+    "v_mfma_f32_16x16x32_f16 a[92:95], v[188:191], v[136:139], 0\n\t"
+    "v_mfma_f32_16x16x32_f16 a[96:99], v[160:163], v[140:143], 0\n\t"
+    "ds_read_b128 v[240:243], v125 offset:8192\n\t"
+    "v_mfma_f32_16x16x32_f16 a[100:103], v[164:167], v[140:143], 0\n\t"
+    "v_mfma_f32_16x16x32_f16 a[104:107], v[168:171], v[140:143], 0\n\t"
+    "ds_read_b128 v[244:247], v125 offset:10240\n\t"
+    "v_mfma_f32_16x16x32_f16 a[108:111], v[172:175], v[140:143], 0\n\t"
+    "s_add_u32 m0, %[tmp], 12288\n\t"
+    "s_add_u32 %[soff], %[soff], %[blk]\n\t"
+    "v_mfma_f32_16x16x32_f16 a[112:115], v[176:179], v[140:143], 0\n\t"
+    "ds_read_b128 v[248:251], v125 offset:12288\n\t"
+    "buffer_load_dwordx4 %[ao1], %[rb], %[soff] offen lds\n\t"
+    "v_mfma_f32_16x16x32_f16 a[116:119], v[180:183], v[140:143], 0\n\t"
+    "v_mfma_f32_16x16x32_f16 a[120:123], v[184:187], v[140:143], 0\n\t"
+    "ds_read_b128 v[252:255], v125 offset:14336\n\t"
+    "v_mfma_f32_16x16x32_f16 a[124:127], v[188:191], v[140:143], 0\n\t"
+    "v_mfma_f32_16x16x32_f16 a[128:131], v[160:163], v[144:147], 0\n\t"
+    "v_mfma_f32_16x16x32_f16 a[132:135], v[164:167], v[144:147], 0\n\t"
+    "v_mfma_f32_16x16x32_f16 a[136:139], v[168:171], v[144:147], 0\n\t"
+    "v_mfma_f32_16x16x32_f16 a[140:143], v[172:175], v[144:147], 0\n\t"
+    "s_add_u32 m0, %[tmp], 16384\n\t"
+    "s_add_u32 %[soff], %[soff], %[blk]\n\t"
+    "v_mfma_f32_16x16x32_f16 a[144:147], v[176:179], v[144:147], 0\n\t"
+    "buffer_load_dwordx4 %[ao0], %[rb], %[soff] offen lds\n\t"
+    "v_mfma_f32_16x16x32_f16 a[148:151], v[180:183], v[144:147], 0\n\t"
+    "v_mfma_f32_16x16x32_f16 a[152:155], v[184:187], v[144:147], 0\n\t"
+    "v_mfma_f32_16x16x32_f16 a[156:159], v[188:191], v[144:147], 0\n\t"
+    "v_mfma_f32_16x16x32_f16 a[160:163], v[160:163], v[148:151], 0\n\t"
+    "v_mfma_f32_16x16x32_f16 a[164:167], v[164:167], v[148:151], 0\n\t"
+    "v_mfma_f32_16x16x32_f16 a[168:171], v[168:171], v[148:151], 0\n\t"
+    "v_mfma_f32_16x16x32_f16 a[172:175], v[172:175], v[148:151], 0\n\t"
+    "s_add_u32 m0, %[tmp], 20480\n\t"
+    "s_add_u32 %[soff], %[soff], %[blk]\n\t"
+    "v_mfma_f32_16x16x32_f16 a[176:179], v[176:179], v[148:151], 0\n\t"
+    "buffer_load_dwordx4 %[ao1], %[rb], %[soff] offen lds\n\t"
+    "v_mfma_f32_16x16x32_f16 a[180:183], v[180:183], v[148:151], 0\n\t"
+    "v_mfma_f32_16x16x32_f16 a[184:187], v[184:187], v[148:151], 0\n\t"
+    "v_mfma_f32_16x16x32_f16 a[188:191], v[188:191], v[148:151], 0\n\t"
+    "v_mfma_f32_16x16x32_f16 a[192:195], v[160:163], v[152:155], 0\n\t"
+    "v_mfma_f32_16x16x32_f16 a[196:199], v[164:167], v[152:155], 0\n\t"
+    "v_mfma_f32_16x16x32_f16 a[200:203], v[168:171], v[152:155], 0\n\t"
+    "v_mfma_f32_16x16x32_f16 a[204:207], v[172:175], v[152:155], 0\n\t"
+    "s_add_u32 m0, %[tmp], 24576\n\t"
+    "s_add_u32 %[soff], %[soff], %[blk]\n\t"
+    "v_mfma_f32_16x16x32_f16 a[208:211], v[176:179], v[152:155], 0\n\t"
+    "buffer_load_dwordx4 %[ao0], %[rb], %[soff] offen lds\n\t"
+    "v_mfma_f32_16x16x32_f16 a[212:215], v[180:183], v[152:155], 0\n\t"
+    "v_mfma_f32_16x16x32_f16 a[216:219], v[184:187], v[152:155], 0\n\t"
+    "v_mfma_f32_16x16x32_f16 a[220:223], v[188:191], v[152:155], 0\n\t"
+    "v_mfma_f32_16x16x32_f16 a[224:227], v[160:163], v[156:159], 0\n\t"
+    "v_mfma_f32_16x16x32_f16 a[228:231], v[164:167], v[156:159], 0\n\t"
+    "v_mfma_f32_16x16x32_f16 a[232:235], v[168:171], v[156:159], 0\n\t"
+    "v_mfma_f32_16x16x32_f16 a[236:239], v[172:175], v[156:159], 0\n\t"
+    "s_add_u32 m0, %[tmp], 28672\n\t"
+    "s_add_u32 %[soff], %[soff], %[blk]\n\t"
+    "v_mfma_f32_16x16x32_f16 a[240:243], v[176:179], v[156:159], 0\n\t"
+    "buffer_load_dwordx4 %[ao1], %[rb], %[soff] offen lds\n\t"
+    "v_mfma_f32_16x16x32_f16 a[244:247], v[180:183], v[156:159], 0\n\t"
+    "v_mfma_f32_16x16x32_f16 a[248:251], v[184:187], v[156:159], 0\n\t"
+    "v_mfma_f32_16x16x32_f16 a[252:255], v[188:191], v[156:159], 0\n\t"
+    "s_waitcnt vmcnt(8) lgkmcnt(0)\n\t"
+    "v_mfma_f32_16x16x32_f16 a[0:3], v[224:227], v[192:195], a[0:3]\n\t"
+    "s_barrier\n\t"
+    "v_add_u32_e32 v124, %[anxt], %[ar0]\n\t"
+    "s_add_u32 %[tmp], %[acur], %[wv]\n\t"
+    "v_mfma_f32_16x16x32_f16 a[4:7], v[228:231], v[192:195], a[4:7]\n\t"
+    "v_add_u32_e32 v125, %[b1], %[br0]\n\t"
+    "v_mfma_f32_16x16x32_f16 a[8:11], v[232:235], v[192:195], a[8:11]\n\t"
+    "s_add_u32 m0, %[tmp], 0\n\t"
+    "s_mov_b32 %[soff], %[t2off]\n\t"
+    "v_mfma_f32_16x16x32_f16 a[12:15], v[236:239], v[192:195], a[12:15]\n\t"
+    "buffer_load_dwordx4 %[ao0], %[ra], %[soff] offen lds\n\t"
+    "v_mfma_f32_16x16x32_f16 a[16:19], v[240:243], v[192:195], a[16:19]\n\t"
+    "ds_read_b128 v[128:131], v124 offset:0\n\t"
+    "v_mfma_f32_16x16x32_f16 a[20:23], v[244:247], v[192:195], a[20:23]\n\t"
+    "ds_read_b128 v[132:135], v124 offset:2048\n\t"
+    "v_mfma_f32_16x16x32_f16 a[24:27], v[248:251], v[192:195], a[24:27]\n\t"
+    "ds_read_b128 v[136:139], v124 offset:4096\n\t"
+    "v_mfma_f32_16x16x32_f16 a[28:31], v[252:255], v[192:195], a[28:31]\n\t"
+    "ds_read_b128 v[140:143], v124 offset:6144\n\t"
+    "v_mfma_f32_16x16x32_f16 a[32:35], v[224:227], v[196:199], a[32:35]\n\t"
+    "ds_read_b128 v[144:147], v124 offset:8192\n\t"
+    "v_mfma_f32_16x16x32_f16 a[36:39], v[228:231], v[196:199], a[36:39]\n\t"
+    "s_add_u32 m0, %[tmp], 4096\n\t"
+    "s_add_u32 %[soff], %[soff], %[blk]\n\t"
+    "v_mfma_f32_16x16x32_f16 a[40:43], v[232:235], v[196:199], a[40:43]\n\t"
+    "buffer_load_dwordx4 %[ao1], %[ra], %[soff] offen lds\n\t"
+    "v_mfma_f32_16x16x32_f16 a[44:47], v[236:239], v[196:199], a[44:47]\n\t"
+    "ds_read_b128 v[148:151], v124 offset:10240\n\t"
+    "v_mfma_f32_16x16x32_f16 a[48:51], v[240:243], v[196:199], a[48:51]\n\t"
+    "ds_read_b128 v[152:155], v124 offset:12288\n\t"
+    "v_mfma_f32_16x16x32_f16 a[52:55], v[244:247], v[196:199], a[52:55]\n\t"
+    "ds_read_b128 v[156:159], v124 offset:14336\n\t"
+    "v_mfma_f32_16x16x32_f16 a[56:59], v[248:251], v[196:199], a[56:59]\n\t"
+    "ds_read_b128 v[160:163], v125 offset:0\n\t"
+    "v_mfma_f32_16x16x32_f16 a[60:63], v[252:255], v[196:199], a[60:63]\n\t"
+    "ds_read_b128 v[164:167], v125 offset:2048\n\t"
+    "v_mfma_f32_16x16x32_f16 a[64:67], v[224:227], v[200:203], a[64:67]\n\t"
+    "s_add_u32 m0, %[tmp], 8192\n\t"
+    "s_add_u32 %[soff], %[soff], %[blk]\n\t"
+    "v_mfma_f32_16x16x32_f16 a[68:71], v[228:231], v[200:203], a[68:71]\n\t"
+    "buffer_load_dwordx4 %[ao0], %[ra], %[soff] offen lds\n\t"
+    "v_mfma_f32_16x16x32_f16 a[72:75], v[232:235], v[200:203], a[72:75]\n\t"
+    "ds_read_b128 v[168:171], v125 offset:4096\n\t"
+    "v_mfma_f32_16x16x32_f16 a[76:79], v[236:239], v[200:203], a[76:79]\n\t"
+    "ds_read_b128 v[172:175], v125 offset:6144\n\t"
+    "v_mfma_f32_16x16x32_f16 a[80:83], v[240:243], v[200:203], a[80:83]\n\t"
+    "ds_read_b128 v[176:179], v125 offset:8192\n\t"
+    "v_mfma_f32_16x16x32_f16 a[84:87], v[244:247], v[200:203], a[84:87]\n\t"
+    "ds_read_b128 v[180:183], v125 offset:10240\n\t"
+    "v_mfma_f32_16x16x32_f16 a[88:91], v[248:251], v[200:203], a[88:91]\n\t"
+    "ds_read_b128 v[184:187], v125 offset:12288\n\t"
+    "v_mfma_f32_16x16x32_f16 a[92:95], v[252:255], v[200:203], a[92:95]\n\t"
+    "s_add_u32 m0, %[tmp], 12288\n\t"
+    "s_add_u32 %[soff], %[soff], %[blk]\n\t"
+    "v_mfma_f32_16x16x32_f16 a[96:99], v[224:227], v[204:207], a[96:99]\n\t"
+    "buffer_load_dwordx4 %[ao1], %[ra], %[soff] offen lds\n\t"
+    "v_mfma_f32_16x16x32_f16 a[100:103], v[228:231], v[204:207], a[100:103]\n\t"
+    "ds_read_b128 v[188:191], v125 offset:14336\n\t"
+    "v_mfma_f32_16x16x32_f16 a[104:107], v[232:235], v[204:207], a[104:107]\n\t"
+    "s_mov_b32 %[swp], %[b0]\n\t"
+    "v_mfma_f32_16x16x32_f16 a[108:111], v[236:239], v[204:207], a[108:111]\n\t"
+    "s_mov_b32 %[b0], %[b1]\n\t"
+    "v_mfma_f32_16x16x32_f16 a[112:115], v[240:243], v[204:207], a[112:115]\n\t"
+    "s_mov_b32 %[b1], %[b2]\n\t"
+    "v_mfma_f32_16x16x32_f16 a[116:119], v[244:247], v[204:207], a[116:119]\n\t"
+    "s_mov_b32 %[b2], %[swp]\n\t"
+    "v_mfma_f32_16x16x32_f16 a[120:123], v[248:251], v[204:207], a[120:123]\n\t"
+    "s_add_u32 m0, %[tmp], 16384\n\t"
+    "s_add_u32 %[soff], %[soff], %[blk]\n\t"
+    "v_mfma_f32_16x16x32_f16 a[124:127], v[252:255], v[204:207], a[124:127]\n\t"
+    "buffer_load_dwordx4 %[ao0], %[ra], %[soff] offen lds\n\t"
+    "v_mfma_f32_16x16x32_f16 a[128:131], v[224:227], v[208:211], a[128:131]\n\t"
+    "s_mov_b32 %[swp], %[acur]\n\t"
+    "v_mfma_f32_16x16x32_f16 a[132:135], v[228:231], v[208:211], a[132:135]\n\t"
+    "s_mov_b32 %[acur], %[anxt]\n\t"
+    "v_mfma_f32_16x16x32_f16 a[136:139], v[232:235], v[208:211], a[136:139]\n\t"
+    "s_mov_b32 %[anxt], %[swp]\n\t"
+    "v_mfma_f32_16x16x32_f16 a[140:143], v[236:239], v[208:211], a[140:143]\n\t"
+    "s_add_u32 %[swp], %[t], 3\n\t"
+    "v_mfma_f32_16x16x32_f16 a[144:147], v[240:243], v[208:211], a[144:147]\n\t"
+    "s_cmp_ge_u32 %[swp], %[kt]\n\t"
+    "s_cselect_b32 %[t2off], %[kt], 0\n\t"
+    "s_cselect_b32 %[sel], %[stgn], %[stg]\n\t"
+    "s_cselect_b32 %[t2offb], %[obn], %[ob]\n\t"
+    "s_cselect_b32 %[sela], %[oan], %[oa]\n\t"
+    "v_mfma_f32_16x16x32_f16 a[148:151], v[244:247], v[208:211], a[148:151]\n\t"
+    "s_add_u32 m0, %[tmp], 20480\n\t"
+    "s_add_u32 %[soff], %[soff], %[blk]\n\t"
+    "v_mfma_f32_16x16x32_f16 a[152:155], v[248:251], v[208:211], a[152:155]\n\t"
+    "buffer_load_dwordx4 %[ao1], %[ra], %[soff] offen lds\n\t"
+    "v_mfma_f32_16x16x32_f16 a[156:159], v[252:255], v[208:211], a[156:159]\n\t"
+    "s_sub_u32 %[swp], %[swp], %[t2off]\n\t"
+    "v_mfma_f32_16x16x32_f16 a[160:163], v[224:227], v[212:215], a[160:163]\n\t"
+    "s_add_u32 %[swp], %[swp], %[sel]\n\t"
+    "v_mfma_f32_16x16x32_f16 a[164:167], v[228:231], v[212:215], a[164:167]\n\t"
+    "s_cmp_ge_u32 %[swp], %[kt]\n\t"
+    "s_cselect_b32 %[t2off], %[kt], 0\n\t"
+    "v_mfma_f32_16x16x32_f16 a[168:171], v[232:235], v[212:215], a[168:171]\n\t"
+    "s_sub_u32 %[swp], %[swp], %[t2off]\n\t"
+    "v_mfma_f32_16x16x32_f16 a[172:175], v[236:239], v[212:215], a[172:175]\n\t"
+    "s_lshl_b32 %[swp], %[swp], 7\n\t"
+    "v_mfma_f32_16x16x32_f16 a[176:179], v[240:243], v[212:215], a[176:179]\n\t"
+    "s_add_u32 m0, %[tmp], 24576\n\t"
+    "s_add_u32 %[soff], %[soff], %[blk]\n\t"
+    "v_mfma_f32_16x16x32_f16 a[180:183], v[244:247], v[212:215], a[180:183]\n\t"
+    "buffer_load_dwordx4 %[ao0], %[ra], %[soff] offen lds\n\t"
+    "v_mfma_f32_16x16x32_f16 a[184:187], v[248:251], v[212:215], a[184:187]\n\t"
+    "s_add_u32 %[t2off], %[swp], %[sela]\n\t"
+    "v_mfma_f32_16x16x32_f16 a[188:191], v[252:255], v[212:215], a[188:191]\n\t"
+    "s_add_u32 %[t2offb], %[swp], %[t2offb]\n\t"
+    "v_mfma_f32_16x16x32_f16 a[192:195], v[224:227], v[216:219], a[192:195]\n\t"
+    "v_add_u32_e32 v124, %[acur], %[ar1]\n\t"
+    "v_mfma_f32_16x16x32_f16 a[196:199], v[228:231], v[216:219], a[196:199]\n\t"
+    "v_add_u32_e32 v125, %[b0], %[br1]\n\t"
+    "v_mfma_f32_16x16x32_f16 a[200:203], v[232:235], v[216:219], a[200:203]\n\t"
+    "v_mfma_f32_16x16x32_f16 a[204:207], v[236:239], v[216:219], a[204:207]\n\t"
+    "s_add_u32 m0, %[tmp], 28672\n\t"
+    "s_add_u32 %[soff], %[soff], %[blk]\n\t"
+    "v_mfma_f32_16x16x32_f16 a[208:211], v[240:243], v[216:219], a[208:211]\n\t"
+    "buffer_load_dwordx4 %[ao1], %[ra], %[soff] offen lds\n\t"
+    "v_mfma_f32_16x16x32_f16 a[212:215], v[244:247], v[216:219], a[212:215]\n\t"
+    "v_mfma_f32_16x16x32_f16 a[216:219], v[248:251], v[216:219], a[216:219]\n\t"
+    "v_mfma_f32_16x16x32_f16 a[220:223], v[252:255], v[216:219], a[220:223]\n\t"
+    "v_mfma_f32_16x16x32_f16 a[224:227], v[224:227], v[220:223], a[224:227]\n\t"
+    "v_mfma_f32_16x16x32_f16 a[228:231], v[228:231], v[220:223], a[228:231]\n\t"
+    "v_mfma_f32_16x16x32_f16 a[232:235], v[232:235], v[220:223], a[232:235]\n\t"
+    "v_mfma_f32_16x16x32_f16 a[236:239], v[236:239], v[220:223], a[236:239]\n\t"
+    "v_mfma_f32_16x16x32_f16 a[240:243], v[240:243], v[220:223], a[240:243]\n\t"
+    "v_mfma_f32_16x16x32_f16 a[244:247], v[244:247], v[220:223], a[244:247]\n\t"
+    "v_mfma_f32_16x16x32_f16 a[248:251], v[248:251], v[220:223], a[248:251]\n\t"
+    "s_add_u32 %[t], %[t], 1\n\t"
+    "s_cmp_lt_u32 %[t], %[kt]\n\t"
+    "v_mfma_f32_16x16x32_f16 a[252:255], v[252:255], v[220:223], a[252:255]\n\t"
+    ".Lw4y_loop_%=:\n\t"
+    "s_waitcnt lgkmcnt(0)\n\t"
+    "v_mfma_f32_16x16x32_f16 a[0:3], v[160:163], v[128:131], a[0:3]\n\t"
+    "ds_read_b128 v[192:195], v124 offset:0\n\t"
+    "v_mfma_f32_16x16x32_f16 a[4:7], v[164:167], v[128:131], a[4:7]\n\t"
+    "v_mfma_f32_16x16x32_f16 a[8:11], v[168:171], v[128:131], a[8:11]\n\t"
+    "ds_read_b128 v[196:199], v124 offset:2048\n\t"
+    "s_add_u32 %[tmp], %[b2], %[wv]\n\t"
+    "v_mfma_f32_16x16x32_f16 a[12:15], v[172:175], v[128:131], a[12:15]\n\t"
+    "s_add_u32 m0, %[tmp], 0\n\t"
+    "s_mov_b32 %[soff], %[t2offb]\n\t"
+    "v_mfma_f32_16x16x32_f16 a[16:19], v[176:179], v[128:131], a[16:19]\n\t"
+    "ds_read_b128 v[200:203], v124 offset:4096\n\t"
+    "buffer_load_dwordx4 %[ao0], %[rb], %[soff] offen lds\n\t"
+    "v_mfma_f32_16x16x32_f16 a[20:23], v[180:183], v[128:131], a[20:23]\n\t"
+    "v_mfma_f32_16x16x32_f16 a[24:27], v[184:187], v[128:131], a[24:27]\n\t"
+    "ds_read_b128 v[204:207], v124 offset:6144\n\t"
+    "v_mfma_f32_16x16x32_f16 a[28:31], v[188:191], v[128:131], a[28:31]\n\t"
+    "v_mfma_f32_16x16x32_f16 a[32:35], v[160:163], v[132:135], a[32:35]\n\t"
+    "ds_read_b128 v[208:211], v124 offset:8192\n\t"
+    "v_mfma_f32_16x16x32_f16 a[36:39], v[164:167], v[132:135], a[36:39]\n\t"
+    "v_mfma_f32_16x16x32_f16 a[40:43], v[168:171], v[132:135], a[40:43]\n\t"
+    "ds_read_b128 v[212:215], v124 offset:10240\n\t"
+    "v_mfma_f32_16x16x32_f16 a[44:47], v[172:175], v[132:135], a[44:47]\n\t"
+    "s_add_u32 m0, %[tmp], 4096\n\t"
+    "s_add_u32 %[soff], %[soff], %[blk]\n\t"
+    "v_mfma_f32_16x16x32_f16 a[48:51], v[176:179], v[132:135], a[48:51]\n\t"
+    "ds_read_b128 v[216:219], v124 offset:12288\n\t"
+    "buffer_load_dwordx4 %[ao1], %[rb], %[soff] offen lds\n\t"
+    "v_mfma_f32_16x16x32_f16 a[52:55], v[180:183], v[132:135], a[52:55]\n\t"
+    "v_mfma_f32_16x16x32_f16 a[56:59], v[184:187], v[132:135], a[56:59]\n\t"
+    "ds_read_b128 v[220:223], v124 offset:14336\n\t"
+    "v_mfma_f32_16x16x32_f16 a[60:63], v[188:191], v[132:135], a[60:63]\n\t"
+    "v_mfma_f32_16x16x32_f16 a[64:67], v[160:163], v[136:139], a[64:67]\n\t"
+    "ds_read_b128 v[224:227], v125 offset:0\n\t"
+    "v_mfma_f32_16x16x32_f16 a[68:71], v[164:167], v[136:139], a[68:71]\n\t"
+    "v_mfma_f32_16x16x32_f16 a[72:75], v[168:171], v[136:139], a[72:75]\n\t"
+    "ds_read_b128 v[228:231], v125 offset:2048\n\t"
+    "v_mfma_f32_16x16x32_f16 a[76:79], v[172:175], v[136:139], a[76:79]\n\t"
+    "s_add_u32 m0, %[tmp], 8192\n\t"
+    "s_add_u32 %[soff], %[soff], %[blk]\n\t"
+    "v_mfma_f32_16x16x32_f16 a[80:83], v[176:179], v[136:139], a[80:83]\n\t"
+    "ds_read_b128 v[232:235], v125 offset:4096\n\t"
+    "buffer_load_dwordx4 %[ao0], %[rb], %[soff] offen lds\n\t"
+    "v_mfma_f32_16x16x32_f16 a[84:87], v[180:183], v[136:139], a[84:87]\n\t"
+    "v_mfma_f32_16x16x32_f16 a[88:91], v[184:187], v[136:139], a[88:91]\n\t"
+    "ds_read_b128 v[236:239], v125 offset:6144\n\t"
+    "v_mfma_f32_16x16x32_f16 a[92:95], v[188:191], v[136:139], a[92:95]\n\t"
+    "v_mfma_f32_16x16x32_f16 a[96:99], v[160:163], v[140:143], a[96:99]\n\t"
+    "ds_read_b128 v[240:243], v125 offset:8192\n\t"
+    "v_mfma_f32_16x16x32_f16 a[100:103], v[164:167], v[140:143], a[100:103]\n\t"
+    "v_mfma_f32_16x16x32_f16 a[104:107], v[168:171], v[140:143], a[104:107]\n\t"
+    "ds_read_b128 v[244:247], v125 offset:10240\n\t"
+    "v_mfma_f32_16x16x32_f16 a[108:111], v[172:175], v[140:143], a[108:111]\n\t"
+    "s_add_u32 m0, %[tmp], 12288\n\t"
+    "s_add_u32 %[soff], %[soff], %[blk]\n\t"
+    "v_mfma_f32_16x16x32_f16 a[112:115], v[176:179], v[140:143], a[112:115]\n\t"
+    "ds_read_b128 v[248:251], v125 offset:12288\n\t"
+    "buffer_load_dwordx4 %[ao1], %[rb], %[soff] offen lds\n\t"
+    "v_mfma_f32_16x16x32_f16 a[116:119], v[180:183], v[140:143], a[116:119]\n\t"
+    "v_mfma_f32_16x16x32_f16 a[120:123], v[184:187], v[140:143], a[120:123]\n\t"
+    "ds_read_b128 v[252:255], v125 offset:14336\n\t"
+    "v_mfma_f32_16x16x32_f16 a[124:127], v[188:191], v[140:143], a[124:127]\n\t"
+    "v_mfma_f32_16x16x32_f16 a[128:131], v[160:163], v[144:147], a[128:131]\n\t"
+    "v_mfma_f32_16x16x32_f16 a[132:135], v[164:167], v[144:147], a[132:135]\n\t"
+    "v_mfma_f32_16x16x32_f16 a[136:139], v[168:171], v[144:147], a[136:139]\n\t"
+    "v_mfma_f32_16x16x32_f16 a[140:143], v[172:175], v[144:147], a[140:143]\n\t"
+    "s_add_u32 m0, %[tmp], 16384\n\t"
+    "s_add_u32 %[soff], %[soff], %[blk]\n\t"
+    "v_mfma_f32_16x16x32_f16 a[144:147], v[176:179], v[144:147], a[144:147]\n\t"
+    "buffer_load_dwordx4 %[ao0], %[rb], %[soff] offen lds\n\t"
+    "v_mfma_f32_16x16x32_f16 a[148:151], v[180:183], v[144:147], a[148:151]\n\t"
+    "v_mfma_f32_16x16x32_f16 a[152:155], v[184:187], v[144:147], a[152:155]\n\t"
+    "v_mfma_f32_16x16x32_f16 a[156:159], v[188:191], v[144:147], a[156:159]\n\t"
+    "v_mfma_f32_16x16x32_f16 a[160:163], v[160:163], v[148:151], a[160:163]\n\t"
+    "v_mfma_f32_16x16x32_f16 a[164:167], v[164:167], v[148:151], a[164:167]\n\t"
+    "v_mfma_f32_16x16x32_f16 a[168:171], v[168:171], v[148:151], a[168:171]\n\t"
+    "v_mfma_f32_16x16x32_f16 a[172:175], v[172:175], v[148:151], a[172:175]\n\t"
+    "s_add_u32 m0, %[tmp], 20480\n\t"
+    "s_add_u32 %[soff], %[soff], %[blk]\n\t"
+    "v_mfma_f32_16x16x32_f16 a[176:179], v[176:179], v[148:151], a[176:179]\n\t"
+    "buffer_load_dwordx4 %[ao1], %[rb], %[soff] offen lds\n\t"
+    "v_mfma_f32_16x16x32_f16 a[180:183], v[180:183], v[148:151], a[180:183]\n\t"
+    "v_mfma_f32_16x16x32_f16 a[184:187], v[184:187], v[148:151], a[184:187]\n\t"
+    "v_mfma_f32_16x16x32_f16 a[188:191], v[188:191], v[148:151], a[188:191]\n\t"
+    "v_mfma_f32_16x16x32_f16 a[192:195], v[160:163], v[152:155], a[192:195]\n\t"
+    "v_mfma_f32_16x16x32_f16 a[196:199], v[164:167], v[152:155], a[196:199]\n\t"
+    "v_mfma_f32_16x16x32_f16 a[200:203], v[168:171], v[152:155], a[200:203]\n\t"
+    "v_mfma_f32_16x16x32_f16 a[204:207], v[172:175], v[152:155], a[204:207]\n\t"
+    "s_add_u32 m0, %[tmp], 24576\n\t"
+    "s_add_u32 %[soff], %[soff], %[blk]\n\t"
+    "v_mfma_f32_16x16x32_f16 a[208:211], v[176:179], v[152:155], a[208:211]\n\t"
+    "buffer_load_dwordx4 %[ao0], %[rb], %[soff] offen lds\n\t"
+    "v_mfma_f32_16x16x32_f16 a[212:215], v[180:183], v[152:155], a[212:215]\n\t"
+    "v_mfma_f32_16x16x32_f16 a[216:219], v[184:187], v[152:155], a[216:219]\n\t"
+    "v_mfma_f32_16x16x32_f16 a[220:223], v[188:191], v[152:155], a[220:223]\n\t"
+    "v_mfma_f32_16x16x32_f16 a[224:227], v[160:163], v[156:159], a[224:227]\n\t"
+    "v_mfma_f32_16x16x32_f16 a[228:231], v[164:167], v[156:159], a[228:231]\n\t"
+    "v_mfma_f32_16x16x32_f16 a[232:235], v[168:171], v[156:159], a[232:235]\n\t"
+    "v_mfma_f32_16x16x32_f16 a[236:239], v[172:175], v[156:159], a[236:239]\n\t"
+    "s_add_u32 m0, %[tmp], 28672\n\t"
+    "s_add_u32 %[soff], %[soff], %[blk]\n\t"
+    "v_mfma_f32_16x16x32_f16 a[240:243], v[176:179], v[156:159], a[240:243]\n\t"
+    "buffer_load_dwordx4 %[ao1], %[rb], %[soff] offen lds\n\t"
+    "v_mfma_f32_16x16x32_f16 a[244:247], v[180:183], v[156:159], a[244:247]\n\t"
+    "v_mfma_f32_16x16x32_f16 a[248:251], v[184:187], v[156:159], a[248:251]\n\t"
+    "v_mfma_f32_16x16x32_f16 a[252:255], v[188:191], v[156:159], a[252:255]\n\t"
+    "s_waitcnt vmcnt(8) lgkmcnt(0)\n\t"
+    "v_mfma_f32_16x16x32_f16 a[0:3], v[224:227], v[192:195], a[0:3]\n\t"
+    "s_barrier\n\t"
+    "v_add_u32_e32 v124, %[anxt], %[ar0]\n\t"
+    "s_add_u32 %[tmp], %[acur], %[wv]\n\t"
+    "v_mfma_f32_16x16x32_f16 a[4:7], v[228:231], v[192:195], a[4:7]\n\t"
+    "v_add_u32_e32 v125, %[b1], %[br0]\n\t"
+    "v_mfma_f32_16x16x32_f16 a[8:11], v[232:235], v[192:195], a[8:11]\n\t"
+    "s_add_u32 m0, %[tmp], 0\n\t"
+    "s_mov_b32 %[soff], %[t2off]\n\t"
+    "v_mfma_f32_16x16x32_f16 a[12:15], v[236:239], v[192:195], a[12:15]\n\t"
+    "buffer_load_dwordx4 %[ao0], %[ra], %[soff] offen lds\n\t"
+    "v_mfma_f32_16x16x32_f16 a[16:19], v[240:243], v[192:195], a[16:19]\n\t"
+    "ds_read_b128 v[128:131], v124 offset:0\n\t"
+    "v_mfma_f32_16x16x32_f16 a[20:23], v[244:247], v[192:195], a[20:23]\n\t"
+    "ds_read_b128 v[132:135], v124 offset:2048\n\t"
+    "v_mfma_f32_16x16x32_f16 a[24:27], v[248:251], v[192:195], a[24:27]\n\t"
+    "ds_read_b128 v[136:139], v124 offset:4096\n\t"
+    "v_mfma_f32_16x16x32_f16 a[28:31], v[252:255], v[192:195], a[28:31]\n\t"
+    "ds_read_b128 v[140:143], v124 offset:6144\n\t"
+    "v_mfma_f32_16x16x32_f16 a[32:35], v[224:227], v[196:199], a[32:35]\n\t"
+    "ds_read_b128 v[144:147], v124 offset:8192\n\t"
+    "v_mfma_f32_16x16x32_f16 a[36:39], v[228:231], v[196:199], a[36:39]\n\t"
+    "s_add_u32 m0, %[tmp], 4096\n\t"
+    "s_add_u32 %[soff], %[soff], %[blk]\n\t"
+    "v_mfma_f32_16x16x32_f16 a[40:43], v[232:235], v[196:199], a[40:43]\n\t"
+    "buffer_load_dwordx4 %[ao1], %[ra], %[soff] offen lds\n\t"
+    "v_mfma_f32_16x16x32_f16 a[44:47], v[236:239], v[196:199], a[44:47]\n\t"
+    "ds_read_b128 v[148:151], v124 offset:10240\n\t"
+    "v_mfma_f32_16x16x32_f16 a[48:51], v[240:243], v[196:199], a[48:51]\n\t"
+    "ds_read_b128 v[152:155], v124 offset:12288\n\t"
+    "v_mfma_f32_16x16x32_f16 a[52:55], v[244:247], v[196:199], a[52:55]\n\t"
+    "ds_read_b128 v[156:159], v124 offset:14336\n\t"
+    "v_mfma_f32_16x16x32_f16 a[56:59], v[248:251], v[196:199], a[56:59]\n\t"
+    "ds_read_b128 v[160:163], v125 offset:0\n\t"
+    "v_mfma_f32_16x16x32_f16 a[60:63], v[252:255], v[196:199], a[60:63]\n\t"
+    "ds_read_b128 v[164:167], v125 offset:2048\n\t"
+    "v_mfma_f32_16x16x32_f16 a[64:67], v[224:227], v[200:203], a[64:67]\n\t"
+    "s_add_u32 m0, %[tmp], 8192\n\t"
+    "s_add_u32 %[soff], %[soff], %[blk]\n\t"
+    "v_mfma_f32_16x16x32_f16 a[68:71], v[228:231], v[200:203], a[68:71]\n\t"
+    "buffer_load_dwordx4 %[ao0], %[ra], %[soff] offen lds\n\t"
+    "v_mfma_f32_16x16x32_f16 a[72:75], v[232:235], v[200:203], a[72:75]\n\t"
+    "ds_read_b128 v[168:171], v125 offset:4096\n\t"
+    "v_mfma_f32_16x16x32_f16 a[76:79], v[236:239], v[200:203], a[76:79]\n\t"
+    "ds_read_b128 v[172:175], v125 offset:6144\n\t"
+    "v_mfma_f32_16x16x32_f16 a[80:83], v[240:243], v[200:203], a[80:83]\n\t"
+    "ds_read_b128 v[176:179], v125 offset:8192\n\t"
+    "v_mfma_f32_16x16x32_f16 a[84:87], v[244:247], v[200:203], a[84:87]\n\t"
+    "ds_read_b128 v[180:183], v125 offset:10240\n\t"
+    "v_mfma_f32_16x16x32_f16 a[88:91], v[248:251], v[200:203], a[88:91]\n\t"
+    "ds_read_b128 v[184:187], v125 offset:12288\n\t"
+    "v_mfma_f32_16x16x32_f16 a[92:95], v[252:255], v[200:203], a[92:95]\n\t"
+    "s_add_u32 m0, %[tmp], 12288\n\t"
+    "s_add_u32 %[soff], %[soff], %[blk]\n\t"
+    "v_mfma_f32_16x16x32_f16 a[96:99], v[224:227], v[204:207], a[96:99]\n\t"
+    "buffer_load_dwordx4 %[ao1], %[ra], %[soff] offen lds\n\t"
+    "v_mfma_f32_16x16x32_f16 a[100:103], v[228:231], v[204:207], a[100:103]\n\t"
+    "ds_read_b128 v[188:191], v125 offset:14336\n\t"
+    "v_mfma_f32_16x16x32_f16 a[104:107], v[232:235], v[204:207], a[104:107]\n\t"
+    "s_mov_b32 %[swp], %[b0]\n\t"
+    "v_mfma_f32_16x16x32_f16 a[108:111], v[236:239], v[204:207], a[108:111]\n\t"
+    "s_mov_b32 %[b0], %[b1]\n\t"
+    "v_mfma_f32_16x16x32_f16 a[112:115], v[240:243], v[204:207], a[112:115]\n\t"
+    "s_mov_b32 %[b1], %[b2]\n\t"
+    "v_mfma_f32_16x16x32_f16 a[116:119], v[244:247], v[204:207], a[116:119]\n\t"
+    "s_mov_b32 %[b2], %[swp]\n\t"
+    "v_mfma_f32_16x16x32_f16 a[120:123], v[248:251], v[204:207], a[120:123]\n\t"
+    "s_add_u32 m0, %[tmp], 16384\n\t"
+    "s_add_u32 %[soff], %[soff], %[blk]\n\t"
+    "v_mfma_f32_16x16x32_f16 a[124:127], v[252:255], v[204:207], a[124:127]\n\t"
+    "buffer_load_dwordx4 %[ao0], %[ra], %[soff] offen lds\n\t"
+    "v_mfma_f32_16x16x32_f16 a[128:131], v[224:227], v[208:211], a[128:131]\n\t"
+    "s_mov_b32 %[swp], %[acur]\n\t"
+    "v_mfma_f32_16x16x32_f16 a[132:135], v[228:231], v[208:211], a[132:135]\n\t"
+    "s_mov_b32 %[acur], %[anxt]\n\t"
+    "v_mfma_f32_16x16x32_f16 a[136:139], v[232:235], v[208:211], a[136:139]\n\t"
+    "s_mov_b32 %[anxt], %[swp]\n\t"
+    "v_mfma_f32_16x16x32_f16 a[140:143], v[236:239], v[208:211], a[140:143]\n\t"
+    "s_add_u32 %[swp], %[t], 3\n\t"
+    "v_mfma_f32_16x16x32_f16 a[144:147], v[240:243], v[208:211], a[144:147]\n\t"
+    "s_cmp_ge_u32 %[swp], %[kt]\n\t"
+    "s_cselect_b32 %[t2off], %[kt], 0\n\t"
+    "s_cselect_b32 %[sel], %[stgn], %[stg]\n\t"
+    "s_cselect_b32 %[t2offb], %[obn], %[ob]\n\t"
+    "s_cselect_b32 %[sela], %[oan], %[oa]\n\t"
+    "v_mfma_f32_16x16x32_f16 a[148:151], v[244:247], v[208:211], a[148:151]\n\t"
+    "s_add_u32 m0, %[tmp], 20480\n\t"
+    "s_add_u32 %[soff], %[soff], %[blk]\n\t"
+    "v_mfma_f32_16x16x32_f16 a[152:155], v[248:251], v[208:211], a[152:155]\n\t"
+    "buffer_load_dwordx4 %[ao1], %[ra], %[soff] offen lds\n\t"
+    "v_mfma_f32_16x16x32_f16 a[156:159], v[252:255], v[208:211], a[156:159]\n\t"
+    "s_sub_u32 %[swp], %[swp], %[t2off]\n\t"
+    "v_mfma_f32_16x16x32_f16 a[160:163], v[224:227], v[212:215], a[160:163]\n\t"
+    "s_add_u32 %[swp], %[swp], %[sel]\n\t"
+    "v_mfma_f32_16x16x32_f16 a[164:167], v[228:231], v[212:215], a[164:167]\n\t"
+    "s_cmp_ge_u32 %[swp], %[kt]\n\t"
+    "s_cselect_b32 %[t2off], %[kt], 0\n\t"
+    "v_mfma_f32_16x16x32_f16 a[168:171], v[232:235], v[212:215], a[168:171]\n\t"
+    "s_sub_u32 %[swp], %[swp], %[t2off]\n\t"
+    "v_mfma_f32_16x16x32_f16 a[172:175], v[236:239], v[212:215], a[172:175]\n\t"
+    "s_lshl_b32 %[swp], %[swp], 7\n\t"
+    "v_mfma_f32_16x16x32_f16 a[176:179], v[240:243], v[212:215], a[176:179]\n\t"
+    "s_add_u32 m0, %[tmp], 24576\n\t"
+    "s_add_u32 %[soff], %[soff], %[blk]\n\t"
+    "v_mfma_f32_16x16x32_f16 a[180:183], v[244:247], v[212:215], a[180:183]\n\t"
+    "buffer_load_dwordx4 %[ao0], %[ra], %[soff] offen lds\n\t"
+    "v_mfma_f32_16x16x32_f16 a[184:187], v[248:251], v[212:215], a[184:187]\n\t"
+    "s_add_u32 %[t2off], %[swp], %[sela]\n\t"
+    "v_mfma_f32_16x16x32_f16 a[188:191], v[252:255], v[212:215], a[188:191]\n\t"
+    "s_add_u32 %[t2offb], %[swp], %[t2offb]\n\t"
+    "v_mfma_f32_16x16x32_f16 a[192:195], v[224:227], v[216:219], a[192:195]\n\t"
+    "v_add_u32_e32 v124, %[acur], %[ar1]\n\t"
+    "v_mfma_f32_16x16x32_f16 a[196:199], v[228:231], v[216:219], a[196:199]\n\t"
+    "v_add_u32_e32 v125, %[b0], %[br1]\n\t"
+    "v_mfma_f32_16x16x32_f16 a[200:203], v[232:235], v[216:219], a[200:203]\n\t"
+    "v_mfma_f32_16x16x32_f16 a[204:207], v[236:239], v[216:219], a[204:207]\n\t"
+    "s_add_u32 m0, %[tmp], 28672\n\t"
+    "s_add_u32 %[soff], %[soff], %[blk]\n\t"
+    "v_mfma_f32_16x16x32_f16 a[208:211], v[240:243], v[216:219], a[208:211]\n\t"
+    "buffer_load_dwordx4 %[ao1], %[ra], %[soff] offen lds\n\t"
+    "v_mfma_f32_16x16x32_f16 a[212:215], v[244:247], v[216:219], a[212:215]\n\t"
+    "v_mfma_f32_16x16x32_f16 a[216:219], v[248:251], v[216:219], a[216:219]\n\t"
+    "v_mfma_f32_16x16x32_f16 a[220:223], v[252:255], v[216:219], a[220:223]\n\t"
+    "v_mfma_f32_16x16x32_f16 a[224:227], v[224:227], v[220:223], a[224:227]\n\t"
+    "v_mfma_f32_16x16x32_f16 a[228:231], v[228:231], v[220:223], a[228:231]\n\t"
+    "v_mfma_f32_16x16x32_f16 a[232:235], v[232:235], v[220:223], a[232:235]\n\t"
+    "v_mfma_f32_16x16x32_f16 a[236:239], v[236:239], v[220:223], a[236:239]\n\t"
+    "v_mfma_f32_16x16x32_f16 a[240:243], v[240:243], v[220:223], a[240:243]\n\t"
+    "v_mfma_f32_16x16x32_f16 a[244:247], v[244:247], v[220:223], a[244:247]\n\t"
+    "v_mfma_f32_16x16x32_f16 a[248:251], v[248:251], v[220:223], a[248:251]\n\t"
+    "s_add_u32 %[t], %[t], 1\n\t"
+    "s_cmp_lt_u32 %[t], %[kt]\n\t"
+    "v_mfma_f32_16x16x32_f16 a[252:255], v[252:255], v[220:223], a[252:255]\n\t"
+    "s_cbranch_scc1 .Lw4y_loop_%=\n\t"
+    "s_waitcnt lgkmcnt(0)\n\t"
+    : [acur] "+s"(w4y_acur), [anxt] "+s"(w4y_anxt), [b0] "+s"(w4y_b0), [b1] "+s"(w4y_b1), [b2] "+s"(w4y_b2),
+      [t] "=&s"(w4y_t), [soff] "=&s"(w4y_soff), [t2off] "=&s"(w4y_t2off), [t2offb] "=&s"(w4y_t2offb), [tmp] "=&s"(w4y_tmp),
+      [swp] "=&s"(w4y_swp), [sel] "=&s"(w4y_sel), [sela] "=&s"(w4y_sela)
+    : [kt] "s"(KT), [stg] "s"(w4y_stg), [stgn] "s"(w4y_stgn), [oa] "s"(w4y_oa), [ob] "s"(w4y_ob), [oan] "s"(w4y_oan),
+      [obn] "s"(w4y_obn), [wv] "s"(w4y_wv), [blk] "s"(w4y_blk), [ra] "s"(w4y_ra), [rb] "s"(w4y_rb),
+      [ao0] "v"(w4y_ao0), [ao1] "v"(w4y_ao1), [ar0] "v"(fr.a_ad[0]), [ar1] "v"(fr.a_ad[1]), [br0] "v"(fr.b_ad[0]),
+      [br1] "v"(fr.b_ad[1])
+    : "memory", "scc", "v124", "v125", "v126", "v127", "v128", "v129", "v130", "v131", "v132", "v133", "v134", "v135", "v136", "v137", "v138", "v139", "v140", "v141", "v142", "v143", "v144", "v145", "v146", "v147", "v148", "v149", "v150", "v151", "v152", "v153", "v154", "v155", "v156", "v157", "v158", "v159", "v160", "v161", "v162", "v163", "v164", "v165", "v166", "v167", "v168", "v169", "v170", "v171", "v172", "v173", "v174", "v175", "v176", "v177", "v178", "v179", "v180", "v181", "v182", "v183", "v184", "v185", "v186", "v187", "v188", "v189", "v190", "v191", "v192", "v193", "v194", "v195", "v196", "v197", "v198", "v199", "v200", "v201", "v202", "v203", "v204", "v205", "v206", "v207", "v208", "v209", "v210", "v211", "v212", "v213", "v214", "v215", "v216", "v217", "v218", "v219", "v220", "v221", "v222", "v223", "v224", "v225", "v226", "v227", "v228", "v229", "v230", "v231", "v232", "v233", "v234", "v235", "v236", "v237", "v238", "v239", "v240", "v241", "v242", "v243", "v244", "v245", "v246", "v247", "v248", "v249", "v250", "v251", "v252", "v253", "v254", "v255", LC_AGPR_ALL);
diff --git a/leetcuda_amd/csrc/lc_knobs.inc b/leetcuda_amd/csrc/lc_knobs.inc
--- a/leetcuda_amd/csrc/lc_knobs.inc
+++ b/leetcuda_amd/csrc/lc_knobs.inc
@@ -13,6 +13,7 @@
 LC_KNOB_SNAP(attn_d512, 0, ok_04, false)
 LC_KNOB_SNAP(w4y_sched, 2, ok_w4y_sched, false)
 LC_KNOB(hgemm_persist, 1, ok_01, false)
+LC_KNOB(hgemm_carry, 1, ok_01, false)
 LC_KNOB(hgemm_stagger, 0, ok_stagger, false)
 LC_KNOB_SNAP(hgemm_tail, 1, ok_04, false)
 LC_KNOB_SNAP(hgemm_tail_tile, 0, ok_02, false)
diff --git a/leetcuda_amd/csrc/lc_launch.h b/leetcuda_amd/csrc/lc_launch.h
--- a/leetcuda_amd/csrc/lc_launch.h
+++ b/leetcuda_amd/csrc/lc_launch.h
@@ -165,6 +165,7 @@
 extern tune_t g_tune_attn_bigd_stagger;
 extern tune_t g_tune_attn_bigd_map;
 extern tune_t g_tune_hgemm_persist;
+extern tune_t g_tune_hgemm_carry;
 extern tune_t g_tune_hgemm_stagger;
 constexpr int STAGGER_OFF = 1 << 27;
 inline int stagger_arg(int kt) {
diff --git a/leetcuda_amd/csrc/tu_w4.hip b/leetcuda_amd/csrc/tu_w4.hip
--- a/leetcuda_amd/csrc/tu_w4.hip
+++ b/leetcuda_amd/csrc/tu_w4.hip
@@ -26,6 +26,16 @@
   } else {
     const int ncu = device_cu_count();
     const bool persist = g_tune_hgemm_persist != 0 && nblk > ncu && nblk % ncu == 0;
+    if constexpr (!B_KN && Y == 2) {
+      const size_t k2 = (size_t)K * 2;
+      if (persist && g_tune_hgemm_carry != 0 && K / BK >= 2 && (size_t)tiles_m * BM * k2 < ((size_t)1 << 31) &&
+          (size_t)tiles_n * BN * k2 < ((size_t)1 << 31)) {
+        auto kc = hgemm_w4y_kernel<false, 2, true>;
+        if (int rc = set_dyn_lds(kc, W4B_LDS)) return rc;
+        hipLaunchKernelGGL(kc, dim3(ncu), dim3(256), W4B_LDS, st, A, B, C, M, N, K, tiles_m, tiles_n, pw, stagger_arg(K / BK), nblk);
+        return check_launch();
+      }
+    }
     hipLaunchKernelGGL(kern, dim3(persist ? ncu : nblk), dim3(256), W4B_LDS, st, A, B, C, M, N, K, tiles_m, tiles_n, pw,
                        stagger_arg(K / BK), persist ? nblk : 0);
   }
```

After: 1530 (median of 6 runs). About the same (+0.8%).
